# Amandaynzhou/CGC-Net

Hardware: AMD Instinct MI355X
Metric: cell-graphs/sec (fwd+bwd), batch=32, ~1800 nodes/16 feat (higher is better)
Workload: dtype f32; 1 GPU; C3: full CGC-Net (3 conv blocks + 2 DiffPool) fwd+bwd+Adam, 32 graphs/GPU/step, ~1803 nodes, ~16159 edges/graph, 16 feat, max_num_nodes=11404 (C1=1140, C2=114), flags=shipped; global_batch=32, nodes_per_batch=57711, parallelism=dp1, includes=CSR build + fwd + loss + bwd + grad all-reduce + Adam, step_sequencer=True, node_order=draw order, fused_adam=True, optimiser=cgc_adam_step (one launch; torch fused Adam arithmetic)

## Files before the change

cgc-net_amd/csrc/exec.hip:

```cpp
#include <stdio.h>
#include <stdlib.h>
#include <string.h>

#include "common.hpp"
#include "groups.hpp"

struct CatArgs {
  const float* src[4];
  int ld[4], width[4], off[4];
};
__global__ __launch_bounds__(256) void k_cat_cols(float* __restrict__ dst, int ldd, long long rows, int total_w, CatArgs a, int nsrc,
                                                  int accumulate) {
  const long long total = rows * total_w;
  for (long long i = blockIdx.x * 256ll + threadIdx.x; i < total; i += (long long)gridDim.x * 256) {
    const long long r = i / total_w;
    const int c = (int)(i - r * total_w);
    int s = 0;
#pragma unroll
    for (int k = 1; k < 4; ++k)
      if (k < nsrc && c >= a.off[k]) s = k;
    const float v = a.src[s][r * a.ld[s] + (c - a.off[s])];
    float* p = dst + r * ldd + c;
    *p = accumulate ? *p + v : v;
  }
}

extern "C" int cgc_cat_cols(float* dst, int ldd, int rows, int nsrc, const float* const* srcs, const int* lds, const int* widths,
                            int accumulate, cgc_stream_t stream) {
  if (nsrc < 1 || nsrc > 4) return CGC_EINVAL;
  CatArgs a;
  int off = 0;
  for (int k = 0; k < 4; ++k) {
    a.src[k] = k < nsrc ? srcs[k] : nullptr;
    a.ld[k] = k < nsrc ? lds[k] : 0;
    a.width[k] = k < nsrc ? widths[k] : 0;
    a.off[k] = off;
    off += a.width[k];
  }
  if (rows <= 0 || off <= 0) return 0;
  const long long total = (long long)rows * off;
  const long long blocks = (total + 255) / 256;
  hipLaunchKernelGGL(k_cat_cols, dim3((unsigned)(blocks < 4096 ? blocks : 4096)), dim3(256), 0, as_stream(stream), dst, ldd,
                     (long long)rows, off, a, nsrc, accumulate);
  CGC_RETURN_IF_LAUNCH_FAILED();
  return 0;
}

__global__ __launch_bounds__(256) void k_transpose(const float* __restrict__ src, int lds, int rows, int cols, float* __restrict__ dst,
                                                   int ldd) {
  __shared__ float t[32][33];
  const int tx = threadIdx.x & 31, ty = threadIdx.x >> 5;
  const int r0 = blockIdx.y * 32, c0 = blockIdx.x * 32;
  for (int j = ty; j < 32; j += 8) {
    const int r = r0 + j, c = c0 + tx;
    if (r < rows && c < cols) t[j][tx] = src[(size_t)r * lds + c];
  }
  __syncthreads();
  for (int j = ty; j < 32; j += 8) {
    const int c = c0 + j, r = r0 + tx;
    if (r < rows && c < cols) dst[(size_t)c * ldd + r] = t[tx][j];
  }
}

extern "C" int cgc_transpose(const float* src, int lds, int rows, int cols, float* dst, int ldd, cgc_stream_t stream) {
  if (rows <= 0 || cols <= 0) return 0;
  hipLaunchKernelGGL(k_transpose, dim3((unsigned)ceil_div(cols, 32), (unsigned)ceil_div(rows, 32)), dim3(256), 0, as_stream(stream), src,
                     lds, rows, cols, dst, ldd);
  CGC_RETURN_IF_LAUNCH_FAILED();
  return 0;
}

int reduce_batch_sum_rows(const float* ws, float* out, int parts, int rows, int width, int ldo, float beta, hipStream_t stream);

namespace {

struct Arena {
  float* base;
  size_t off = 0, high = 0;
  explicit Arena(float* b) : base(b) {}
  float* f(size_t n) {
    off = (off + 63) & ~(size_t)63;
    float* p = base + off;
    off += n;
    if (off > high) high = off;
    return p;
  }
  int* i(size_t n) { return reinterpret_cast<int*>(f(n)); }
  size_t mark() const { return off; }
  void release(size_t m) { off = m; }
};

struct Ctx {
  cgc_stream_t s;
  bool dry;
  Arena* scratch;
  float* gws;
  int64_t gws_floats;
  int gemm_mode = CGC_GEMM_EXACT;
};

static int fail_at(int rc, const char* what, int line) {
  static const bool verbose = getenv("CGC_EXEC_DEBUG") != nullptr;
  if (verbose) fprintf(stderr, "cgc exec.hip:%d: rc %d from %s\n", line, rc, what);
  return rc;
}
#define CALL(expr)                                              \
  do {                                                          \
    if (!c.dry) {                                               \
      const int rc__ = (expr);                                  \
      if (rc__ != 0) return fail_at(rc__, #expr, __LINE__);     \
    }                                                           \
  } while (0)
#define TRY(expr)                                               \
  do {                                                          \
    const int rc__ = (expr);                                    \
    if (rc__ != 0) return fail_at(rc__, #expr, __LINE__);       \
  } while (0)

inline int up(int v, int m) { return (v + m - 1) / m * m; }
inline int wide_ld(int F) { return (F >= 256 && F % 32 != 0) ? up(F, 32) : (F > 32 && F % 4 != 0) ? up(F, 4) : F; }
inline int pad4_ld(int c) { return (c > 32 && c % 4 != 0) ? up(c, 4) : c; }

int gemm(const Ctx& c, int tA, int tB, int M, int N, int K, const float* A, int lda, const float* B, int ldb, float beta, float* C, int ldc,
         const float* bias = nullptr, int batch = 1, int64_t sA = 0, int64_t sB = 0, int64_t sC = 0, const int* gptr = nullptr,
         int ragged = 0, int max_ragged = 0, int nx = 0, const float* const* xA = nullptr, const int* xlda = nullptr,
         const int64_t* xsA = nullptr, const float* const* xB = nullptr, const int* xldb = nullptr, const int64_t* xsB = nullptr,
         const int* xK = nullptr) {
  if (c.dry) return 0;
  return cgc_gemm_f32(tA, tB, M, N, K, 1.f, A, lda, B, ldb, beta, C, ldc, bias, batch, sA, sB, sC, gptr, ragged, max_ragged, nx, xA, xlda,
                      xsA, xB, xldb, xsB, xK, c.gws, c.gws_floats, c.gemm_mode, c.s);
}

int gemm_x1(const Ctx& c, int tA, int tB, int M, int N, int K, const float* A, int lda, const float* B, int ldb, float beta, float* C, int ldc,
            const float* bias, int batch, int64_t sA, int64_t sB, int64_t sC, const int* gptr, int ragged, int max_ragged, const float* xA,
            int xlda, int64_t xsA, const float* xB, int xldb, int64_t xsB, int xK) {
  return gemm(c, tA, tB, M, N, K, A, lda, B, ldb, beta, C, ldc, bias, batch, sA, sB, sC, gptr, ragged, max_ragged, 1, &xA, &xlda, &xsA,
              &xB, &xldb, &xsB, &xK);
}

int split_parts(int Fa, int Fb, int n) {
  const int tm = Fa <= 32 ? 32 : Fa <= 64 ? 64 : 128, tn = Fb <= 32 ? 32 : Fb <= 64 ? 64 : 128;
  const int tiles = ceil_div(Fa, tm) * ceil_div(Fb, tn);
  int best = 1;
  double best_score = -1.0;
  int hi = n / 512;
  if (hi > 128) hi = 128;
  if (hi < 1) hi = 1;
  for (int parts = 1; parts <= hi; ++parts) {
    const int blocks = tiles * parts, rounds = ceil_div(blocks, 512);
    const double fill = (double)blocks / ((double)rounds * 512.0);
    const double score = fill - 0.02 * rounds - (blocks < 256 ? 0.5 : 0.0);
    if (score > best_score + 1e-9) {
      best = parts;
      best_score = score;
    }
  }
  return best;
}

int gemm_tn_rows(const Ctx& c, const float* A, int lda, int Fa, const float* B, int ldb, int Fb, int n, float* out, int ldo = 0) {
  if (ldo <= 0) ldo = Fb;
  int parts = split_parts(Fa, Fb, n);
  if (parts == 1) return gemm(c, 1, 0, Fa, Fb, n, A, lda, B, ldb, 0.f, out, ldo);
  const int chunk = up(ceil_div(n, parts), 32);
  parts = ceil_div(n, chunk);
  const size_t m = c.scratch->mark();
  float* ws = c.scratch->f((size_t)parts * Fa * Fb);
  TRY(gemm(c, 1, 0, Fa, Fb, n, A, lda, B, ldb, 0.f, ws, Fb, nullptr, parts, 0, 0, (int64_t)Fa * Fb, nullptr, 3, chunk));
  CALL(reduce_batch_sum_rows(ws, out, parts, Fa, Fb, ldo, 0.f, as_stream(c.s)));
  c.scratch->release(m);
  return 0;
}

struct T3 {
  float* p;
  int b, r, c, ld;
  int64_t bs() const { return (int64_t)r * ld; }
};

int bgemm(const Ctx& c, const T3& A, const T3& B, const T3& C, int tA, int tB, float beta = 0.f) {
  const int batch = C.b, M = C.r, N = C.c, Kd = tA ? A.r : A.c;
  if (tA && !tB && M <= 128 && N <= 128 && Kd >= 512 && batch * 2 < 256 && C.ld == N) {
    int parts = Kd / 128;
    const int want = ceil_div(384, batch * (N > 64 ? 2 : 1));
    if (want < parts) parts = want;
    if (parts < 2) parts = 2;
    const int step = up(ceil_div(Kd, parts), 32);
    parts = ceil_div(Kd, step);
    const size_t m = c.scratch->mark();
    float* ws = c.scratch->f((size_t)batch * parts * M * N);
    TRY(gemm(c, 1, 0, M, N, Kd, A.p, A.ld, B.p, B.ld, 0.f, ws, N, nullptr, batch * parts, 0, 0, (int64_t)M * N, nullptr, 3, step));
    CALL(cgc_reduce_batched(ws, C.p, batch, parts, M * N, beta, c.s));
    c.scratch->release(m);
    return 0;
  }
  return gemm(c, tA, tB, M, N, Kd, A.p, A.ld, B.p, B.ld, beta, C.p, C.ld, nullptr, batch, A.bs(), B.bs(), C.bs());
}

int cat2(const Ctx& c, float* dst, int ldd, int rows, const float* a, int lda, int wa, const float* b, int ldb, int wb, int accumulate = 0) {
  const float* s[2] = {a, b};
  const int l[2] = {lda, ldb}, w[2] = {wa, wb};
  CALL(cgc_cat_cols(dst, ldd, rows, 2, s, l, w, accumulate, c.s));
  return 0;
}
int cat3(const Ctx& c, float* dst, int ldd, int rows, const float* a, int lda, int wa, const float* b, int ldb, int wb, const float* d, int ldd3,
         int wd) {
  const float* s[3] = {a, b, d};
  const int l[3] = {lda, ldb, ldd3}, w[3] = {wa, wb, wd};
  CALL(cgc_cat_cols(dst, ldd, rows, 3, s, l, w, 0, c.s));
  return 0;
}
int add1(const Ctx& c, float* dst, int ldd, int rows, const float* a, int lda, int wa) {
  const float* s[1] = {a};
  const int l[1] = {lda}, w[1] = {wa};
  CALL(cgc_cat_cols(dst, ldd, rows, 1, s, l, w, 1, c.s));
  return 0;
}

struct LayerP {
  const float *W, *b, *gamma, *beta;
  float *rm, *rv;
  int64_t* nbt;
  float eps, mom;
};
struct LayerS {
  float *hn, *rinv, *mean, *istd;
};

inline LayerP layer_params(const cgc_level_desc& d, const cgc_block_params* p, int k, int slot) {
  LayerP r;
  r.W = p->W[k];
  r.b = d.has_bias ? p->b[k] : nullptr;
  r.gamma = d.has_bn ? p->gamma[k] : nullptr;
  r.beta = d.has_bn ? p->beta[k] : nullptr;
  r.rm = d.has_bn ? p->running_mean[k] : nullptr;
  r.rv = d.has_bn ? p->running_var[k] : nullptr;
  r.nbt = d.has_bn ? p->num_batches_tracked[k] : nullptr;
  r.eps = d.bn_eps[slot];
  r.mom = d.bn_momentum[slot];
  return r;
}

inline size_t stats_ws_floats(int n, int F) { return (size_t)cgc_stats_ws_floats(n, F); }

int layer_fwd(const Ctx& c, const cgc_level_desc& d, const LayerP& p, const LayerS& s, const float* agg, int lda, int n, int fin, int F,
              float* y, int ldy, float* y2 = nullptr, int ldy2 = 0) {
  const size_t m = c.scratch->mark();
  const int batch_stats = d.has_bn && !d.eval;
  float* ws = batch_stats ? c.scratch->f(stats_ws_floats(n, F)) : nullptr;
  int fused = 0;
  if ((F >= 256 || F <= 32) && fin <= 32 && !c.dry) {
    int rc;
    if (F <= 32)
      rc = cgc_sage_narrow_fwd(agg, lda, p.W, p.b, n, fin, F, 1, d.act, s.hn, s.rinv, batch_stats, ws, d.count, p.eps, p.mom, p.rm, p.rv, p.nbt,
                               s.mean, s.istd, c.s);
    else
      rc = cgc_sage_wide_fwd(agg, lda, p.W, p.b, n, fin, F, 1, d.act, s.hn, F, s.rinv, batch_stats, ws, d.count, p.eps, p.mom, p.rm, p.rv, p.nbt,
                             s.mean, s.istd, c.s);
    if (rc == 0) fused = 1;
    else if (rc != CGC_EINVAL) return rc;
  }
  if (!fused) {
    TRY(gemm(c, 0, 0, n, F, fin, agg, lda, p.W, F, 0.f, s.hn, F, p.b));
    if (batch_stats)
      CALL(cgc_l2norm_act_bn(s.hn, n, F, 1, d.act, s.hn, s.rinv, ws, d.count, p.eps, p.mom, p.rm, p.rv, p.nbt, s.mean, s.istd, c.s));
    else
      CALL(cgc_l2norm_act_stats(s.hn, n, F, 1, d.act, s.hn, s.rinv, nullptr, nullptr, c.s));
  }
  if (d.has_bn && d.eval) CALL(cgc_bn_running_stats(p.rm, p.rv, F, p.eps, s.mean, s.istd, c.s));
  CALL(cgc_bn_act_apply(s.hn, n, F, d.act, d.has_bn ? s.mean : nullptr, s.istd, p.gamma, p.beta, y, ldy, y2, ldy2, c.s));
  c.scratch->release(m);
  return 0;
}

int layer_bwd(const Ctx& c, const cgc_level_desc& d, const LayerP& p, const LayerS& s, const float* agg, int lda, int n, int fin, int F,
              const float* dy, int ldy, float* dagg, int ldd, float* dwdb, float* sums) {
  const size_t m = c.scratch->mark();
  const int mode = d.has_bn ? 2 : 0;
  const size_t slot_floats = (size_t)(cgc_stats_blocks(n, F) > 1 ? cgc_stats_blocks(n, F) : 1) * 2 * F;
  if (d.has_bn) {
    float* ws = c.scratch->f(slot_floats);
    CALL(cgc_bn_bwd_reduce(dy, ldy, s.hn, n, F, d.act, s.mean, s.istd, sums, ws, c.s));
  }
  float* db = d.has_bias ? dwdb + (size_t)fin * F : nullptr;
  if (F <= 32 && fin <= 32) {
    float* ws = c.scratch->f((size_t)cgc_sage_narrow_ws_floats(n, fin, F));
    CALL(cgc_sage_narrow_bwd(dy, ldy, s.hn, s.rinv, n, F, d.act, 1, mode, s.mean, s.istd, p.gamma, d.has_bn ? sums : nullptr, d.count, agg,
                             lda, fin, p.W, dagg, ldd, dwdb, ws, c.s));
  } else {
    float* dh = c.scratch->f((size_t)n * F);
    float* ws = db ? c.scratch->f(slot_floats) : nullptr;
    CALL(cgc_bn_act_l2_bwd(dy, ldy, s.hn, s.rinv, n, F, d.act, 1, mode, s.mean, s.istd, p.gamma, d.has_bn ? sums : nullptr, d.count, dh, db, ws,
                           c.s));
    if (dagg) TRY(gemm(c, 0, 1, n, fin, F, dh, F, p.W, F, 0.f, dagg, ldd));
    TRY(gemm_tn_rows(c, agg, lda, fin, dh, F, F, n, dwdb));
  }
  c.scratch->release(m);
  return 0;
}

inline bool pairable(int fin_e, int F_e, int fin_p, int F_p) { return fin_e == fin_p && F_e == F_p && fin_e <= 32 && F_e <= 32; }

int layer_fwd_pair(const Ctx& c, const cgc_level_desc& d, const LayerP* p, const LayerS* s, const float* const* agg, int lda, int n, int fin, int F,
                   float* const* y, int ldy, float* const* y2, const int* ldy2) {
  const size_t m = c.scratch->mark();
  SnFwdPtrs g[2];
  SnFwdBn bn[2];
  BnApplyPtrs ap[2];
  const int batch_stats = d.has_bn && !d.eval;
  for (int i = 0; i < 2; ++i) {
    float* ws = batch_stats ? c.scratch->f(stats_ws_floats(n, F)) : nullptr;
    g[i] = SnFwdPtrs{agg[i], p[i].W, p[i].b, s[i].hn, s[i].rinv, ws};
    bn[i] = SnFwdBn{p[i].eps, p[i].mom, p[i].rm, p[i].rv, p[i].nbt, s[i].mean, s[i].istd};
    ap[i] = BnApplyPtrs{s[i].hn, d.has_bn ? s[i].mean : nullptr, s[i].istd, p[i].gamma, p[i].beta, y[i], y2[i], ldy2[i]};
  }
  CALL(sage_narrow_fwd_groups(g, bn, 2, lda, n, fin, F, 1, d.act, batch_stats, d.count, as_stream(c.s)));
  if (d.has_bn && d.eval)
    for (int i = 0; i < 2; ++i) CALL(cgc_bn_running_stats(p[i].rm, p[i].rv, F, p[i].eps, s[i].mean, s[i].istd, c.s));
  CALL(bn_act_apply_groups(ap, 2, n, F, d.act, ldy, as_stream(c.s)));
  c.scratch->release(m);
  return 0;
}

int layer_bwd_pair(const Ctx& c, const cgc_level_desc& d, const LayerP* p, const LayerS* s, const float* const* agg, int lda, int n, int fin, int F,
                   const float* const* dy, int ldy, float* const* dagg, int ldd, float* const* dwdb, float* const* sums) {
  const size_t m = c.scratch->mark();
  const int mode = d.has_bn ? 2 : 0;
  const size_t slot_floats = (size_t)(cgc_stats_blocks(n, F) > 1 ? cgc_stats_blocks(n, F) : 1) * 2 * F;
  if (d.has_bn) {
    BnRedPtrs r[2];
    for (int i = 0; i < 2; ++i) r[i] = BnRedPtrs{dy[i], s[i].hn, s[i].mean, s[i].istd, c.scratch->f(slot_floats)};
    CALL(bn_bwd_reduce_groups(r, sums, 2, ldy, n, F, d.act, as_stream(c.s)));
  }
  SnBwdPtrs g[2];
  for (int i = 0; i < 2; ++i)
    g[i] = SnBwdPtrs{dy[i], s[i].hn, s[i].rinv, s[i].mean, s[i].istd, p[i].gamma, d.has_bn ? sums[i] : nullptr, agg[i], p[i].W, dagg[i],
                     c.scratch->f((size_t)cgc_sage_narrow_ws_floats(n, fin, F))};
  CALL(sage_narrow_bwd_groups(g, dwdb, 2, ldy, n, F, d.act, 1, mode, d.count, lda, fin, ldd, as_stream(c.s)));
  c.scratch->release(m);
  return 0;
}

struct Level {
  const cgc_level_desc& d;
  int n, B, R, fin, H, E, AH, C, D, D3, wp, wt, ldp, ldC, ldP, ldW, ftot, npad_jk, seg_nmax;
  bool dense, pool, tall;
  float *At, *An, *invd, *ge1, *agg0, *pair[2], *xcat, *aggk[2], *hp3, *cat_e, *HS, *CS, *jk_out, *x12, *S, *P;
  float *G, *keep;
  bool reg;
  double reg_numel, reg_rows;
  int* arg;
  LayerS L[6];
  cgc_level_grad_layout gl;

  explicit Level(const cgc_level_desc& dd) : d(dd) {
    n = d.n; B = d.B; R = d.rows_per_graph; fin = d.fin; H = d.H; E = d.E; AH = d.AH; C = d.C;
    dense = d.level >= 2;
    pool = C > 0;
    D3 = 2 * H + E;
    D = d.jk ? H : D3;
    wp = pool ? H + AH : H;
    wt = 2 * wp + fin;
    ldp = dense ? wt : wp;
    ldC = pool ? wide_ld(C) : 0;
    ldP = dense ? pad4_ld(C) : ldC;
    ftot = 2 * AH + C;
    tall = pool && n >= 8 * C;
    ldW = wide_ld(C);
    npad_jk = up(n > 1 ? n : 1, 1024);
    seg_nmax = dense ? R : d.npad;
    reg = pool && (d.flags & 8);
    const double N = dense ? R : d.npad;
    reg_numel = (double)B * N * N;
    reg_rows = (double)B * N;
    memset(&gl, 0, sizeof(gl));
  }

  void layout_saved(Arena& a) {
    At = An = invd = ge1 = nullptr;
    if (dense) {
      if (d.renorm) At = a.f((size_t)n * R);
      An = a.f((size_t)n * R);
      invd = a.f(n);
      ge1 = a.f(n);
    }
    agg0 = a.f((size_t)n * fin);
    xcat = dense ? a.f((size_t)n * wt) : nullptr;
    for (int k = 0; k < 2; ++k) {
      pair[k] = dense ? xcat + (1 - k) * wp : a.f((size_t)n * wp);
      aggk[k] = a.f((size_t)n * wp);
    }
    hp3 = pool ? a.f((size_t)n * ldC) : nullptr;
    for (int k = 0; k < 6; ++k) {
      const bool emb = k < 3;
      if (!emb && !pool) {
        L[k].hn = L[k].rinv = L[k].mean = L[k].istd = nullptr;
        continue;
      }
      const int F = width_out(k);
      L[k].hn = a.f((size_t)n * F);
      L[k].rinv = a.f(n);
      L[k].mean = a.f(F);
      L[k].istd = a.f(F);
    }
    cat_e = a.f((size_t)n * D3);
    HS = CS = jk_out = nullptr;
    if (d.jk) {
      const int Hh = 3 * H / 2;
      HS = a.f((size_t)6 * Hh * npad_jk);
      CS = a.f((size_t)6 * Hh * npad_jk);
      jk_out = a.f((size_t)n * H);
    }
    arg = a.i((size_t)B * D);
    x12 = S = P = nullptr;
    if (pool) {
      x12 = a.f((size_t)n * 2 * AH);
      S = a.f((size_t)n * ldC);
      P = a.f((size_t)n * ldP);
    }
    G = keep = nullptr;
    if (reg) {
// ... 84 lines not shown
  TRY(aggregate(c, L, g, gptr, x_in, L.fin, L.fin, L.agg0));
  if (L.dense) {
    const float* s1[1] = {x_in};
    const int l1[1] = {L.fin}, w1[1] = {L.fin};
    CALL(cgc_cat_cols(L.xcat + 2 * wp, L.wt, n, 1, s1, l1, w1, 0, c.s));
  }
  for (int k = 0; k < 3; ++k) {
    const float* ain = k == 0 ? L.agg0 : L.aggk[k - 1];
    const int lda = k == 0 ? L.fin : wp;
    if (k < 2 && L.pool && pairable(L.width_in(k), H, L.width_in(3 + k), AH)) {
      const LayerP pp[2] = {layer_params(d, emb, k, k), layer_params(d, pl, k, 3 + k)};
      const LayerS ss[2] = {L.L[k], L.L[3 + k]};
      const float* ag[2] = {ain, k == 0 ? ain : ain + H};
      float* yy[2] = {L.pair[k], L.pair[k] + H};
      float* y2[2] = {L.cat_e + k * H, L.x12 + k * AH};
      const int l2[2] = {L.D3, 2 * AH};
      TRY(layer_fwd_pair(c, d, pp, ss, ag, lda, n, L.width_in(k), H, yy, L.ldp, y2, l2));
      if (k < 2) TRY(aggregate(c, L, g, gptr, L.pair[k], L.ldp, wp, L.aggk[k]));
      continue;
    }
    if (k < 2)
      TRY(layer_fwd(c, d, layer_params(d, emb, k, k), L.L[k], ain, lda, n, L.width_in(k), L.width_out(k), L.pair[k], L.ldp, L.cat_e + k * H,
                    L.D3));
    else
      TRY(layer_fwd(c, d, layer_params(d, emb, k, k), L.L[k], ain, lda, n, L.width_in(k), L.width_out(k), L.cat_e + 2 * H, L.D3));
    if (L.pool) {
      const float* ainp = k == 0 ? ain : ain + H;
      if (k < 2)
        TRY(layer_fwd(c, d, layer_params(d, pl, k, 3 + k), L.L[3 + k], ainp, lda, n, L.width_in(3 + k), L.width_out(3 + k), L.pair[k] + H, L.ldp,
                      L.x12 + k * AH, 2 * AH));
      else
        TRY(layer_fwd(c, d, layer_params(d, pl, k, 3 + k), L.L[3 + k], ainp, lda, n, L.width_in(3 + k), L.width_out(3 + k), L.hp3, L.ldC));
    }
    if (k < 2) TRY(aggregate(c, L, g, gptr, L.pair[k], L.ldp, wp, L.aggk[k]));
  }
  if (d.jk) CALL(cgc_jk_lstm_fwd(L.cat_e, n, L.npad_jk, H, jk->lstm, jk->w_att, jk->b_att, L.jk_out, L.HS, L.CS, c.s));
  CALL(cgc_segment_max_fwd(L.embed(), gptr, L.B, L.D, L.seg_nmax, readout, L.arg, c.s));
  if (!L.pool) return 0;
  {
    const bool wide_main = C > 2 * AH;
    const float* xm = wide_main ? L.hp3 : L.x12;
    const float* xe = wide_main ? L.x12 : L.hp3;
    const int ldm = wide_main ? L.ldC : 2 * AH, lde = wide_main ? 2 * AH : L.ldC;
    const int wm = wide_main ? C : 2 * AH, we = wide_main ? 2 * AH : C;
    const int om = wide_main ? 2 * AH : 0, oe = wide_main ? 0 : 2 * AH;
    if (L.tall) {
      const size_t m = c.scratch->mark();
      float* wt = c.scratch->f((size_t)L.ftot * L.ldW);
      CALL(cgc_transpose(pl->lin_W, L.ftot, C, L.ftot, wt, L.ldW, c.s));
      TRY(gemm_x1(c, 0, 0, n, C, wm, xm, ldm, wt + (size_t)om * L.ldW, L.ldW, 0.f, L.S, L.ldC, pl->lin_b, 1, 0, 0, 0, nullptr, 0, 0, xe, lde, 0,
                  wt + (size_t)oe * L.ldW, L.ldW, 0, we));
      c.scratch->release(m);
    } else {
      TRY(gemm_x1(c, 0, 1, n, C, wm, xm, ldm, pl->lin_W + om, L.ftot, 0.f, L.S, L.ldC, pl->lin_b, 1, 0, 0, 0, nullptr, 0, 0, xe, lde, 0,
                  pl->lin_W + oe, L.ftot, 0, we));
    }
  }
  CALL(cgc_softmax_fwd(L.S, n, C, L.ldC, L.S, c.s));
  if (!L.dense) {
    CALL(cgc_spmm_graphs(g->rowptr, g->col, nullptr, g->val, nullptr, nullptr, L.S, L.P, n, C, L.ldC, gptr, L.B, d.nmax, 1 | (g->spatial ? 4 : 0), g->gorder, c.s));
    TRY(gemm(c, 1, 0, C, L.D, 0, L.S, L.ldC, L.embed(), L.D, 0.f, x_out, L.D, nullptr, L.B, 0, 0, (int64_t)C * L.D, gptr, 2, d.nmax));
    TRY(gemm(c, 1, 0, C, C, 0, L.S, L.ldC, L.P, L.ldC, 0.f, A_out, C, nullptr, L.B, 0, 0, (int64_t)C * C, gptr, 2, d.nmax));
  } else {
    const T3 s3{L.S, L.B, L.R, C, L.ldC}, e3{const_cast<float*>(L.embed()), L.B, L.R, L.D, L.D}, p3{L.P, L.B, L.R, C, L.ldP};
    const T3 a3{const_cast<float*>(d.renorm ? L.At : A_in), L.B, L.R, L.R, L.R};
    TRY(bgemm(c, s3, e3, T3{x_out, L.B, C, L.D, L.D}, 1, 0));
    TRY(bgemm(c, a3, s3, p3, 0, 0));
    TRY(bgemm(c, s3, p3, T3{A_out, L.B, C, C, C}, 1, 0));
  }
  if (L.reg) TRY(reg_fwd(c, L, g, gptr, A_in, A_out, reg_out));
  return 0;
}

int level_bwd_blocks(const Ctx& c, Level& L, const cgc_block_params* emb, const cgc_block_params* pl, const cgc_jk_params* jk,
                     const cgc_graph* g, const int* gptr, const float* x_in, const float* A_in, float* d_embed, const float* dx12,
                     float* dagg1, const float* gAt, float* grads, float* d_x_in, float* d_A_in) {
  const cgc_level_desc& d = L.d;
  Arena& sc = *c.scratch;
  const int n = L.n, H = L.H, AH = L.AH, wp = L.wp, B = L.B, R = L.R, D3 = L.D3, fin = L.fin;
  auto sums = [&](int k) { return grads + L.gl.W[k] + (int64_t)L.width_in(k) * L.width_out(k) + L.width_out(k); };
  float* d_cat = d_embed;
  if (d.jk) {
    d_cat = sc.f((size_t)n * D3);
    const size_t m = sc.mark();
    float* ws = sc.f((size_t)cgc_jk_bwd_ws_floats(H));
    CALL(cgc_jk_lstm_bwd_flat(L.cat_e, d_embed, n, L.npad_jk, H, jk->lstm, jk->w_att, jk->b_att, L.HS, L.CS, d_cat, grads + L.gl.jk, ws, c.s));
    sc.release(m);
  }
  float* dagg[2];
  const int ldg = L.ldp;
  float* const gcat = dagg1 != nullptr ? dagg1 : sc.f((size_t)n * ldg);
  dagg[1] = gcat;
  TRY(layer_bwd(c, d, layer_params(d, emb, 2, 2), L.L[2], L.aggk[1], wp, n, H, L.E, d_cat + 2 * H, D3, dagg[1], ldg, grads + L.gl.W[2], sums(2)));
  float* dpair = nullptr;
  for (int k = 1; k >= 0; --k) {
    dpair = sc.f((size_t)n * wp);
    TRY(aggregate_t(c, L, g, gptr, dagg[k], ldg, wp, dpair));
    if (L.pool) TRY(cat2(c, dpair, wp, n, d_cat + k * H, D3, H, dx12 + k * AH, 2 * AH, AH, 1));
    else TRY(add1(c, dpair, wp, n, d_cat + k * H, D3, H));
    const bool first = k == 0;
    const bool need_in = !first || L.dense;
    const float* ain = first ? L.agg0 : L.aggk[k - 1];
    const int lda = first ? fin : wp;
    const int fi_e = L.width_in(k), fi_p = L.width_in(3 + k);
    float *de = nullptr, *dp = nullptr;
    int ldd = ldg;
    if (need_in && !first) {
      de = dagg[0] = L.dense ? gcat + wp : sc.f((size_t)n * wp);
      dp = de + H;
    } else if (need_in) {
      de = gcat + 2 * wp;
      dp = L.pool ? sc.f((size_t)n * ldg) : nullptr;
    }
    if (L.pool && pairable(fi_e, H, fi_p, AH)) {
      const LayerP pp[2] = {layer_params(d, emb, k, k), layer_params(d, pl, k, 3 + k)};
      const LayerS ss[2] = {L.L[k], L.L[3 + k]};
      const float* ag[2] = {ain, first ? ain : ain + H};
      const float* dyy[2] = {dpair, dpair + H};
      float* dg[2] = {de, dp};
      float* dw[2] = {grads + L.gl.W[k], grads + L.gl.W[3 + k]};
      float* sm[2] = {sums(k), sums(3 + k)};
      TRY(layer_bwd_pair(c, d, pp, ss, ag, lda, n, fi_e, H, dyy, wp, dg, ldd, dw, sm));
    } else {
      TRY(layer_bwd(c, d, layer_params(d, emb, k, k), L.L[k], ain, lda, n, fi_e, H, dpair, wp, de, ldd, grads + L.gl.W[k], sums(k)));
      if (L.pool)
        TRY(layer_bwd(c, d, layer_params(d, pl, k, 3 + k), L.L[3 + k], first ? ain : ain + H, lda, n, fi_p, AH, dpair + H, wp, dp, ldd,
                      grads + L.gl.W[3 + k], sums(3 + k)));
    }
    if (first && L.dense) {
      if (L.pool) TRY(add1(c, de, ldg, n, dp, ldg, fin));
      TRY(aggregate_t(c, L, g, gptr, de, ldg, fin, d_x_in));
      float* dAn = sc.f((size_t)n * R);
      TRY(bgemm(c, T3{gcat, B, R, L.wt, L.wt}, T3{L.xcat, B, R, L.wt, L.wt}, T3{dAn, B, R, R, R}, 0, 1));
      CALL(cgc_adj_prep_bwd(A_in, L.An, L.invd, L.ge1, dAn, gAt, n, R, d.renorm ? d.renorm_p : -1.f, d_A_in, c.s));
    }
  }
  return 0;
}

int level_bwd(const Ctx& c, Level& L, const cgc_block_params* emb, const cgc_block_params* pl, const cgc_jk_params* jk, const cgc_graph* g,
              const int* gptr, const float* x_in, const float* A_in, const float* d_readout, const float* d_xo, const float* d_ao, float* grads,
              float* d_x_in, float* d_A_in, const float* d_reg = nullptr) {
  const cgc_level_desc& d = L.d;
  Arena& sc = *c.scratch;
  const int n = L.n, H = L.H, AH = L.AH, wp = L.wp, C = L.C, D = L.D, B = L.B, R = L.R;
  float* d_embed = sc.f((size_t)n * D);
  CALL(cgc_segment_max_bwd_full(d_readout, L.arg, gptr, B, D, L.seg_nmax, d_embed, c.s));
  float *dx12 = nullptr, *gAt = nullptr;
  if (L.pool) {
    float *Gs = nullptr, *coef = nullptr;
    if (L.reg) {
      float* dao = sc.f((size_t)B * C * C);
      Gs = sc.f((size_t)B * C * C);
      coef = sc.f(4);
      CALL(cgc_diffpool_reg_bwd_prep(d_reg, L.keep, L.reg_numel, L.reg_rows, d_ao, dao, L.G, Gs, B, C, coef, c.s));
      d_ao = dao;
    }
    const size_t m0 = sc.mark();
    float* ds = sc.f((size_t)n * L.ldC);
    if (!L.dense) {
      float* dp = sc.f((size_t)n * L.ldC);
      TRY(gemm(c, 0, 0, 0, C, C, L.S, L.ldC, d_ao, C, 0.f, dp, L.ldC, nullptr, B, 0, (int64_t)C * C, 0, gptr, 1, d.nmax));
      CALL(cgc_spmm_graphs(g->t_rowptr, g->t_col, nullptr, g->t_val, nullptr, nullptr, dp, ds, n, C, L.ldC, gptr, B, d.nmax, 2 | (g->spatial ? 4 : 0), g->gorder,
                           c.s));
      TRY(gemm_x1(c, 0, 1, 0, C, C, L.P, L.ldC, d_ao, C, 1.f, ds, L.ldC, nullptr, B, 0, (int64_t)C * C, 0, gptr, 1, d.nmax, L.embed(), D, 0, d_xo,
                  D, (int64_t)C * D, D));
      if (L.reg) TRY(gemm(c, 0, 0, 0, C, C, L.S, L.ldC, Gs, C, 1.f, ds, L.ldC, nullptr, B, 0, (int64_t)C * C, 0, gptr, 1, d.nmax));
      TRY(gemm(c, 0, 0, 0, D, C, L.S, L.ldC, d_xo, D, 1.f, d_embed, D, nullptr, B, 0, (int64_t)C * D, 0, gptr, 1, d.nmax));
    } else {
      gAt = sc.f((size_t)n * R);
      float* dP = sc.f((size_t)n * L.ldP);
      const T3 s3{L.S, B, R, C, L.ldC}, e3{const_cast<float*>(L.embed()), B, R, D, D}, p3{L.P, B, R, C, L.ldP};
      const T3 a3{const_cast<float*>(d.renorm ? L.At : A_in), B, R, R, R};
      const T3 dao{const_cast<float*>(d_ao), B, C, C, C}, dxo{const_cast<float*>(d_xo), B, C, D, D};
      const T3 ds3{ds, B, R, C, L.ldC}, dP3{dP, B, R, C, L.ldP};
      TRY(bgemm(c, p3, dao, ds3, 0, 1));
      TRY(bgemm(c, s3, dao, dP3, 0, 0));
      TRY(bgemm(c, dP3, s3, T3{gAt, B, R, R, R}, 0, 1));
      TRY(bgemm(c, a3, dP3, ds3, 1, 0, 1.f));
      TRY(bgemm(c, e3, dxo, ds3, 0, 1, 1.f));
      TRY(bgemm(c, s3, dxo, T3{d_embed, B, R, D, D}, 0, 0, 1.f));
      if (L.reg) {
        TRY(bgemm(c, s3, T3{Gs, B, C, C, C}, ds3, 0, 0, 1.f));
        CALL(cgc_diffpool_reg_adj_bwd(a3.p, (int64_t)n * R, coef, gAt, 1, c.s));
      }
    }
    if (L.reg) CALL(cgc_diffpool_reg_entropy_bwd(L.S, n, C, L.ldC, coef, ds, L.ldC, c.s));
    float* dz = sc.f((size_t)n * L.ldC);
    {
      const size_t m = sc.mark();
      float* ws = sc.f((size_t)(cgc_stats_blocks(n, C) > 1 ? cgc_stats_blocks(n, C) : 1) * 2 * C);
      CALL(cgc_softmax_bwd(L.S, ds, n, C, L.ldC, dz, grads + L.gl.lin_b, ws, c.s));
      sc.release(m);
    }
    dx12 = sc.f((size_t)n * 2 * AH);
    float* dy3 = sc.f((size_t)n * L.ldC);
    TRY(gemm(c, 0, 0, n, 2 * AH, C, dz, L.ldC, pl->lin_W, L.ftot, 0.f, dx12, 2 * AH));
    TRY(gemm(c, 0, 0, n, C, C, dz, L.ldC, pl->lin_W + 2 * AH, L.ftot, 0.f, dy3, L.ldC));
    {
      float* dW = grads + L.gl.lin_W;
      TRY(gemm_tn_rows(c, dz, L.ldC, C, L.x12, 2 * AH, 2 * AH, n, dW, L.ftot));
      TRY(gemm_tn_rows(c, dz, L.ldC, C, L.hp3, L.ldC, C, n, dW + 2 * AH, L.ftot));
    }
    (void)m0;
    float* dagg1 = sc.f((size_t)n * L.ldp);
    TRY(layer_bwd(c, d, layer_params(d, pl, 2, 5), L.L[5], L.aggk[1] + H, wp, n, AH, C, dy3, L.ldC, dagg1 + H, L.ldp, grads + L.gl.W[5],
                  grads + L.gl.W[5] + (int64_t)AH * C + C));
    return level_bwd_blocks(c, L, emb, pl, jk, g, gptr, x_in, A_in, d_embed, dx12, dagg1, gAt, grads, d_x_in, d_A_in);
  }
  return level_bwd_blocks(c, L, emb, pl, jk, g, gptr, x_in, A_in, d_embed, nullptr, nullptr, nullptr, grads, d_x_in, d_A_in);
}

template <class Body>
int run_level(const cgc_level_desc* d, float* saved, float* scratch, cgc_stream_t stream, Body&& body) {
  Level L(*d);
  Arena sv(saved), sc(scratch);
  L.layout_saved(sv);
  L.layout_grads();
  Ctx c{stream, false, &sc, nullptr, cgc_gemm_ws_floats()};
  c.gws = sc.f((size_t)c.gws_floats);
  c.gemm_mode = (d->flags & 2) ? CGC_GEMM_SPLIT_BF16 : (d->flags & 4) ? CGC_GEMM_SPLIT_F16 : CGC_GEMM_EXACT;
  return body(c, L);
}

}

extern "C" int cgc_level_supported(const cgc_level_desc* d) {
  if (d == nullptr || d->level < 1 || d->level > 3 || d->B < 1 || d->B > 65535 || d->n < 1) return 0;
  if (d->fin < 1 || d->H < 1 || d->E < 1 || d->act < 0 || d->act > 3) return 0;
  if (d->level >= 2 && (d->rows_per_graph < 1 || (long long)d->B * d->rows_per_graph != d->n)) return 0;
  if (d->level == 1 && (d->nmax < 1 || d->npad < d->nmax)) return 0;
  if (d->C > 0 && (d->AH < 1 || d->H + d->AH > 256 || (2 * d->AH) % 4 != 0)) return 0;
  if (d->C == 0 && d->level == 1) return 0;
  if ((d->flags & ~14) || (d->flags & 6) == 6) return 0;
  if ((d->flags & 8) && d->C == 0) return 0;
  if (d->jk && (d->E != d->H || !cgc_jk_matrix_core(d->H))) return 0;
  return 1;
}

extern "C" int64_t cgc_level_saved_floats(const cgc_level_desc* d) {
  if (!cgc_level_supported(d)) return -1;
  Level L(*d);
  Arena a(nullptr);
  L.layout_saved(a);
  return (int64_t)a.high + 64;
}

extern "C" int cgc_level_grad_layout_of(const cgc_level_desc* d, cgc_level_grad_layout* out) {
  if (!cgc_level_supported(d) || out == nullptr) return CGC_EINVAL;
  Level L(*d);
  L.layout_grads();
  *out = L.gl;
  return 0;
}

extern "C" int64_t cgc_level_scratch_floats(const cgc_level_desc* d) {
  if (!cgc_level_supported(d)) return -1;
  Level L(*d);
  Arena sv(nullptr);
  L.layout_saved(sv);
  L.layout_grads();
  size_t high = 0;
  for (int pass = 0; pass < (d->eval ? 1 : 2); ++pass) {
    Arena sc(nullptr);
    Ctx c{nullptr, true, &sc, nullptr, 0};
    sc.f((size_t)cgc_gemm_ws_floats());
    cgc_block_params bp;
    memset(&bp, 0, sizeof(bp));
    cgc_jk_params jp;
    memset(&jp, 0, sizeof(jp));
    cgc_graph gr;
    memset(&gr, 0, sizeof(gr));
    const int rc = pass == 0 ? level_fwd(c, L, &bp, &bp, &jp, &gr, nullptr, nullptr, nullptr, nullptr, nullptr, nullptr)
                             : level_bwd(c, L, &bp, &bp, &jp, &gr, nullptr, nullptr, nullptr, nullptr, nullptr, nullptr, nullptr, nullptr, nullptr);
    if (rc != 0) return -1;
    if (sc.high > high) high = sc.high;
  }
  return (int64_t)high + 64;
}

extern "C" int cgc_level_fwd(const cgc_level_desc* d, const cgc_block_params* emb, const cgc_block_params* pool, const cgc_jk_params* jk,
                             const cgc_graph* g, const int* gptr, const float* x_in, const float* A_in, float* saved, float* scratch,
                             float* readout, float* x_out, float* A_out, const float** assign_out, int* assign_ld, float* reg_out,
                             cgc_stream_t stream) {
  if (!cgc_level_supported(d) || saved == nullptr || scratch == nullptr) return CGC_EINVAL;
  if (!aligned16(saved) || !aligned16(scratch)) return CGC_EINVAL;
  if ((d->flags & 8) && reg_out == nullptr) return CGC_EINVAL;
  return run_level(d, saved, scratch, stream, [&](const Ctx& c, Level& L) {
    const int rc = level_fwd(c, L, emb, pool, jk, g, gptr, x_in, A_in, readout, x_out, A_out, reg_out);
    if (assign_out != nullptr) *assign_out = L.S;
    if (assign_ld != nullptr) *assign_ld = L.ldC;
    return rc;
  });
}

extern "C" int cgc_level_bwd(const cgc_level_desc* d, const cgc_block_params* emb, const cgc_block_params* pool, const cgc_jk_params* jk,
                             const cgc_graph* g, const int* gptr, const float* x_in, const float* A_in, const float* saved, float* scratch,
                             const float* d_readout, const float* d_x_out, const float* d_A_out, const float* d_reg, float* grads,
                             float* d_x_in, float* d_A_in, cgc_stream_t stream) {
  if (!cgc_level_supported(d) || saved == nullptr || scratch == nullptr || grads == nullptr || d->eval) return CGC_EINVAL;
  if (!aligned16(saved) || !aligned16(scratch) || !aligned16(grads)) return CGC_EINVAL;
  if ((d->flags & 8) && d_reg == nullptr) return CGC_EINVAL;
  return run_level(d, const_cast<float*>(saved), scratch, stream, [&](const Ctx& c, Level& L) {
    return level_bwd(c, L, emb, pool, jk, g, gptr, x_in, A_in, d_readout, d_x_out, d_A_out, grads, d_x_in, d_A_in, d_reg);
  });
}
```

cgc-net_amd/csrc/gemm.hip:

```cpp
#include "gemm_common.hpp"

template <int ROWS>
struct KContigLoader {
  static constexpr int UNITS = ROWS * (BK / 4);
  static constexpr int PER_T = (UNITS + 255) / 256;
  float4 reg[PER_T];
  __device__ __forceinline__ void load(const float* __restrict__ base, int ld, int row0, int row_lim, int k0, int k_lim, bool vec_ok) {
#pragma unroll
    for (int i = 0; i < PER_T; ++i) {
      const int u = threadIdx.x + i * 256;
      float4 v = make_float4(0.f, 0.f, 0.f, 0.f);
      if (UNITS % 256 == 0 || u < UNITS) {
        const int row = row0 + u / (BK / 4);
        const int k = k0 + (u % (BK / 4)) * 4;
        if (row < row_lim && k < k_lim) {
          const float* p = base + (size_t)row * ld + k;
          if (vec_ok && k + 3 < k_lim) {
            v = *reinterpret_cast<const float4*>(p);
          } else {
            v.x = p[0];
            if (k + 1 < k_lim) v.y = p[1];
            if (k + 2 < k_lim) v.z = p[2];
            if (k + 3 < k_lim) v.w = p[3];
          }
        }
      }
      reg[i] = v;
    }
  }
  __device__ __forceinline__ void load_fast(const float* __restrict__ base, int ld, int row0, int row_last, int k0) {
#pragma unroll
    for (int i = 0; i < PER_T; ++i) {
      const int u = threadIdx.x + i * 256;
      const int row = min(row0 + u / (BK / 4), row_last);
      reg[i] = *reinterpret_cast<const float4*>(base + (size_t)row * ld + k0 + (u % (BK / 4)) * 4);
    }
  }
  __device__ __forceinline__ void offsets(unsigned (&off)[PER_T], int ld, int row0, int row_last) const {
#pragma unroll
    for (int i = 0; i < PER_T; ++i) {
      const int u = threadIdx.x + i * 256;
      off[i] = (unsigned)min(row0 + u / (BK / 4), row_last) * (unsigned)ld * 4u + (unsigned)(u % (BK / 4)) * 16u;
    }
  }
  static __device__ __forceinline__ unsigned tile_soffset(int , int k0) { return (unsigned)k0 * 4u; }
  __device__ __forceinline__ void load_buf_part(int i, __amdgpu_buffer_rsrc_t rsrc, const unsigned (&off)[PER_T], unsigned soff) {
    reg[i] = __builtin_bit_cast(float4, __builtin_amdgcn_raw_buffer_load_b128(rsrc, off[i], soff, 0));
  }
  __device__ __forceinline__ void load_fast_masked(const float* __restrict__ base, int ld, int row0, int row_last, int k0, int k_lim) {
    const int k_last4 = (k_lim - 1) & ~3;
#pragma unroll
    for (int i = 0; i < PER_T; ++i) {
      const int u = threadIdx.x + i * 256;
      const int row = min(row0 + u / (BK / 4), row_last);
      const int k = k0 + (u % (BK / 4)) * 4;
      float4 v = *reinterpret_cast<const float4*>(base + (size_t)row * ld + min(k, k_last4));
      if (k >= k_lim) v.x = 0.f;
      if (k + 1 >= k_lim) v.y = 0.f;
      if (k + 2 >= k_lim) v.z = 0.f;
      if (k + 3 >= k_lim) v.w = 0.f;
      reg[i] = v;
    }
  }
  __device__ __forceinline__ void store_part(int i, float* __restrict__ lds) const {
    const int u = threadIdx.x + i * 256;
    if (UNITS % 256 == 0 || u < UNITS)
      *reinterpret_cast<float4*>(&lds[(u / (BK / 4)) * KC_LD + (u % (BK / 4)) * 4]) = reg[i];
  }
  __device__ __forceinline__ void store(float* __restrict__ lds) const {
#pragma unroll
    for (int i = 0; i < PER_T; ++i) store_part(i, lds);
  }
};

template <int COLS>
struct MnContigLoader {
  static constexpr int UNITS = BK * (COLS / 4);
  static constexpr int PER_T = (UNITS + 255) / 256;
  float4 reg[PER_T];
  __device__ __forceinline__ void load(const float* __restrict__ base, int ld, int col0, int col_lim, int k0, int k_lim, bool vec_ok) {
#pragma unroll
    for (int i = 0; i < PER_T; ++i) {
      const int u = threadIdx.x + i * 256;
// ... 484 lines not shown
  if (batch <= 0 || N <= 0) return 0;
  if (ragged == 1 && (transA || a.gptr == nullptr)) return CGC_EINVAL;
  if (ragged == 2 && (!transA || transB || a.gptr == nullptr || a.nx > 0)) return CGC_EINVAL;
  if (ragged == 3 && (!transA || transB || a.nx > 0 || max_ragged <= 0 || K <= 0 || batch % ceil_div(K, max_ragged) != 0)) return CGC_EINVAL;
  if (ragged < 0 || ragged > 3) return CGC_EINVAL;
  a.chunk = ragged == 3 ? max_ragged : 0;
  const int m_extent = ragged == 1 ? max_ragged : M;
  if (m_extent <= 0) return 0;
  const int k_extent = ragged >= 2 ? max_ragged : K;
  constexpr int shortk_max = 160, fill_min = 448;
  const bool sk = k_extent <= shortk_max && a.nx == 0;
  const long long fill = (long long)ceil_div(m_extent, 128) * batch;
  const bool want_split = mode == CGC_GEMM_SPLIT_BF16, want_half = mode == CGC_GEMM_SPLIT_F16;
  auto big_route = [&](bool shortk, float* w) -> int {
    if ((want_split || want_half) && !shortk && !(transA && transB) && gemm_all_fast(a, transA, transB, batch, m_extent, k_extent)) {
      int rc = want_half ? gemm_half_launch(a, transA, transB, batch, m_extent, k_extent, w, ws_floats, stream) : CGC_EINVAL;
      if (rc == CGC_EINVAL) rc = gemm_split_launch(a, transA, transB, batch, m_extent, k_extent, w, ws_floats, stream);
      if (rc != CGC_EINVAL) return rc;
    }
    return launch_cfg<2, 2, 2, 2>(a, transA, transB, batch, m_extent, k_extent, shortk, w, ws_floats, stream);
  };
  const int force = g_force_cfg;
  if (force > 0) {
    const bool fsk = force >= 20 ? true : force >= 10 ? false : sk;
    switch (force % 10) {
      case 1: return big_route(fsk, ws);
      case 2: return launch_cfg<4, 1, 1, 2>(a, transA, transB, batch, m_extent, k_extent, fsk, ws, ws_floats, stream);
      case 3: return launch_cfg<1, 4, 2, 1>(a, transA, transB, batch, m_extent, k_extent, fsk, ws, ws_floats, stream);
      case 4: return launch_cfg<2, 2, 1, 1>(a, transA, transB, batch, m_extent, k_extent, fsk, ws, ws_floats, stream);
      case 5: return launch_cfg<4, 1, 1, 1>(a, transA, transB, batch, m_extent, k_extent, fsk, ws, ws_floats, stream);
      case 6: return launch_cfg<1, 4, 1, 1>(a, transA, transB, batch, m_extent, k_extent, fsk, ws, ws_floats, stream);
      default: break;
    }
  }
  if (N <= 32) return launch_cfg<4, 1, 1, 1>(a, transA, transB, batch, m_extent, k_extent, sk, ws, ws_floats, stream);
  if (N <= 64) {
    if (m_extent > 64 && fill < fill_min) return launch_cfg<2, 2, 1, 1>(a, transA, transB, batch, m_extent, k_extent, sk, ws, ws_floats, stream);
    return launch_cfg<4, 1, 1, 2>(a, transA, transB, batch, m_extent, k_extent, sk, ws, ws_floats, stream);
  }
  if (m_extent <= 32) return launch_cfg<1, 4, 1, 1>(a, transA, transB, batch, m_extent, k_extent, sk, ws, ws_floats, stream);
  if (m_extent <= 64) return launch_cfg<1, 4, 2, 1>(a, transA, transB, batch, m_extent, k_extent, sk, ws, ws_floats, stream);
  if (fill * ceil_div(N, 128) < fill_min) {
    if (N <= 128) {
      if (k_extent > 256 && m_extent > 128)
        return launch_cfg<4, 1, 1, 1>(a, transA, transB, batch, m_extent, k_extent, sk, ws, ws_floats, stream);
      return launch_cfg<2, 2, 1, 1>(a, transA, transB, batch, m_extent, k_extent, sk, ws, ws_floats, stream);
    }
    if (transA) {
      if (!sk && ws != nullptr && k_extent >= 24 * BK) return big_route(sk, ws);
      return launch_cfg<4, 1, 1, 2>(a, transA, transB, batch, m_extent, k_extent, sk, ws, ws_floats, stream);
    }
    return launch_cfg<1, 4, 2, 1>(a, transA, transB, batch, m_extent, k_extent, sk, ws, ws_floats, stream);
  }
  return big_route(sk, ws);
}

extern "C" int cgc_gemm_f32(int transA, int transB, int M, int N, int K, float alpha, const float* A, int lda, const float* B, int ldb,
                            float beta, float* C, int ldc, const float* bias, int batch, int64_t strideA, int64_t strideB,
                            int64_t strideC, const int* gptr, int ragged, int max_ragged, int nx, const float* const* xA,
                            const int* xlda, const int64_t* xstrideA, const float* const* xB, const int* xldb,
                            const int64_t* xstrideB, const int* xK, float* ws, int64_t ws_floats, int mode, cgc_stream_t stream_) {
  if (nx < 0 || nx > 2) return CGC_EINVAL;
  if (mode != CGC_GEMM_EXACT && mode != CGC_GEMM_SPLIT_BF16 && mode != CGC_GEMM_SPLIT_F16) return CGC_EINVAL;
  GemmArgs a;
  a.A = A; a.B = B; a.C = C; a.bias = bias; a.gptr = gptr;
  a.M = M; a.N = N; a.K = K; a.lda = lda; a.ldb = ldb; a.ldc = ldc;
  a.strideA = strideA; a.strideB = strideB; a.strideC = strideC;
  a.alpha = alpha; a.beta = beta; a.ragged = ragged; a.tiles_n = 0;
  a.per_batch = a.nb = 0; a.ws = nullptr; a.resident = 0; a.s_max = 1; a.chunk = 0; a.scale = nullptr;
  for (int i = 0; i < 2; ++i) { a.xA[i] = a.xB[i] = nullptr; a.xlda[i] = a.xldb[i] = a.xK[i] = 0; a.xsA[i] = a.xsB[i] = 0; }
  int kept = 0;
  for (int i = 0; i < nx; ++i) {
    if (xK[i] <= 0) continue;
    a.xA[kept] = xA[i]; a.xB[kept] = xB[i]; a.xlda[kept] = xlda[i]; a.xldb[kept] = xldb[i]; a.xK[kept] = xK[i];
    a.xsA[kept] = xstrideA[i]; a.xsB[kept] = xstrideB[i];
    ++kept;
  }
  a.nx = kept;
  return gemm_dispatch(a, transA, transB, batch, max_ragged, ws, ws_floats, mode, as_stream(stream_));
}

__global__ void k_reduce_batch_sum(const float* __restrict__ ws, float* __restrict__ out, int parts, long long numel, float beta, int width,
                                   int ldo) {
  for (long long i = blockIdx.x * (long long)blockDim.x + threadIdx.x; i < numel; i += (long long)gridDim.x * blockDim.x) {
    float s = 0.f;
    for (int p = 0; p < parts; ++p) s += ws[(size_t)p * numel + i];
    const long long o = (i / width) * ldo + i % width;
    out[o] = beta != 0.f ? s + beta * out[o] : s;
  }
}

__global__ __launch_bounds__(256) void k_reduce_many_parts(const float* __restrict__ ws, float* __restrict__ out, int parts, int numel,
                                                           float beta, int width, int ldo) {
  __shared__ float part[8][32];
  const int cl = threadIdx.x & 31, grp = threadIdx.x >> 5;
  const int c = blockIdx.x * 32 + cl;
  ws += (size_t)blockIdx.y * parts * numel;
  out += (size_t)blockIdx.y * numel;
  float s = 0.f;
  if (c < numel) {
    float a[8];
#pragma unroll
    for (int u = 0; u < 8; ++u) a[u] = 0.f;
    int k = grp;
    for (; k + 56 < parts; k += 64) {
#pragma unroll
      for (int u = 0; u < 8; ++u) a[u] += ws[(size_t)(k + 8 * u) * numel + c];
    }
    for (; k < parts; k += 8) a[0] += ws[(size_t)k * numel + c];
    s = ((a[0] + a[1]) + (a[2] + a[3])) + ((a[4] + a[5]) + (a[6] + a[7]));
  }
  part[grp][cl] = s;
  __syncthreads();
  if (grp == 0 && c < numel) {
    float t = part[0][cl];
#pragma unroll
    for (int g = 1; g < 8; ++g) t += part[g][cl];
    const int o = (c / width) * ldo + c % width;
    out[o] = beta != 0.f ? t + beta * out[o] : t;
  }
}

extern "C" int cgc_reduce_batched(const float* ws, float* out, int outer, int parts, int numel, float beta, cgc_stream_t stream) {
  if (numel <= 0 || outer <= 0) return 0;
  if (outer > 65535) return CGC_EINVAL;
  hipLaunchKernelGGL(k_reduce_many_parts, dim3((unsigned)ceil_div(numel, 32), (unsigned)outer), dim3(256), 0, as_stream(stream), ws, out,
                     parts, numel, beta, numel, numel);
  CGC_RETURN_IF_LAUNCH_FAILED();
  return 0;
}

int reduce_batch_sum_rows(const float* ws, float* out, int parts, int rows, int width, int ldo, float beta, hipStream_t stream) {
  const int64_t numel = (int64_t)rows * width;
  if (numel <= 0) return 0;
  if (width <= 0 || ldo < width || numel > 0x7fffffff) return CGC_EINVAL;
  if (parts >= 16 && numel <= (1 << 20)) {
    hipLaunchKernelGGL(k_reduce_many_parts, dim3((unsigned)ceil_div((int)numel, 32), 1u), dim3(256), 0, stream, ws, out, parts, (int)numel, beta,
                       width, ldo);
  } else {
    const int64_t blocks = ceil_div64(numel, 256);
    hipLaunchKernelGGL(k_reduce_batch_sum, dim3((unsigned)(blocks < 4096 ? blocks : 4096)), dim3(256), 0, stream, ws, out, parts,
                       (long long)numel, beta, width, ldo);
  }
  CGC_RETURN_IF_LAUNCH_FAILED();
  return 0;
}

extern "C" int cgc_reduce_batch_sum(const float* ws, float* out, int parts, int64_t numel, float beta, cgc_stream_t stream) {
  if (numel <= 0) return 0;
  if (parts >= 16 && numel <= (1 << 20)) return cgc_reduce_batched(ws, out, 1, parts, (int)numel, beta, stream);
  const int64_t blocks = ceil_div64(numel, 256);
  const int w = numel <= 0x7fffffff ? (int)numel : 0x7fffffff;
  hipLaunchKernelGGL(k_reduce_batch_sum, dim3((unsigned)(blocks < 4096 ? blocks : 4096)), dim3(256), 0, as_stream(stream), ws, out,
                     parts, (long long)numel, beta, w, w);
  CGC_RETURN_IF_LAUNCH_FAILED();
  return 0;
}
```

cgc-net_amd/csrc/groups.hpp:

```cpp
#pragma once
#include "common.hpp"

struct SnFwdPtrs {
  const float *agg, *W, *bias;
  float *hn, *rinv, *ws;
};
struct SnFwdBn {
  float eps, momentum;
  float *running_mean, *running_var;
  int64_t* nbt;
  float *mean, *istd;
};
struct SnBwdPtrs {
  const float *dy, *hn, *rinv, *mean, *istd, *gamma, *sums, *agg, *W;
  float *dagg, *ws;
};
struct StatsFinPtrs {
  const float* ws;
  float *running_mean, *running_var, *mean, *istd;
  long long* nbt;
  float eps, momentum;
};
struct BnApplyPtrs {
  const float *hn, *mean, *istd, *gamma, *beta;
  float *y, *y2;
  int ldy2;
};
struct BnRedPtrs {
  const float *dy, *hn, *mean, *istd;
  float* ws;
};

int sage_narrow_fwd_groups(const SnFwdPtrs* g, const SnFwdBn* bn, int ng, int lda, int n, int K, int F, int normalize, int act, int stats,
                           double count, hipStream_t st);
int sage_narrow_bwd_groups(const SnBwdPtrs* g, float* const* dwdb, int ng, int ldy, int n, int F, int act, int normalize, int mode, double count,
                           int lda, int fin, int ldd, hipStream_t st);
int bn_act_apply_groups(const BnApplyPtrs* g, int ng, int n, int F, int act, int ldy, hipStream_t stream);
int bn_bwd_reduce_groups(const BnRedPtrs* g, float* const* sums, int ng, int ldy, int n, int F, int act, hipStream_t stream);
int launch_stats_finalize_groups(const StatsFinPtrs* g, int ng, int slots, int F, double count, hipStream_t stream);
int launch_reduce_slots_f32_pair(const float* ws0, float* out0, const float* ws1, float* out1, int ng, int slots, int width, hipStream_t stream);
```

cgc-net_amd/csrc/jk.hip:

```cpp
#include "jk.hpp"

template <int C>
__device__ __forceinline__ void jk_fill_lds(const JkWeights& w, float4* Wt, float4* B4, float* watt, int nthreads) {
  constexpr int H = JkDims<C>::H, KIN = JkDims<C>::KIN;
  for (int idx = threadIdx.x; idx < 2 * H * KIN; idx += nthreads) {
    const int d = idx / (H * KIN), rem = idx - d * H * KIN, j = rem / KIN, k = rem - j * KIN;
    float v[4];
#pragma unroll
    for (int g = 0; g < 4; ++g) {
      const int row = g * H + j;
      v[g] = k < C ? w.w_ih[d][row * C + k] : w.w_hh[d][row * H + (k - C)];
    }
    Wt[idx] = make_float4(v[0], v[1], v[2], v[3]);
  }
  for (int idx = threadIdx.x; idx < 2 * H; idx += nthreads) {
    const int d = idx / H, j = idx - d * H;
    float v[4];
#pragma unroll
    for (int g = 0; g < 4; ++g) v[g] = w.b_ih[d][g * H + j] + w.b_hh[d][g * H + j];
    B4[idx] = make_float4(v[0], v[1], v[2], v[3]);
    watt[idx] = w.w_att[idx];
  }
  if (threadIdx.x == 0) watt[2 * H] = w.b_att[0];
}
// ... 255 lines not shown
extern "C" int cgc_jk_matrix_core(int C) { return C == 4 || C == 8 || C == 12 || C == 16 || C == 20; }

#define JK_FOR_EACH_C(X) X(2) X(4) X(6) X(8) X(10) X(12) X(14) X(16) X(18) X(20) X(22) X(24) X(26) X(28) X(30) X(32)

template <int C>
static void jk_allow_lds() {
  static bool done_f[CGC_MAX_DEVICES] = {}, done_b[CGC_MAX_DEVICES] = {};
  cgc_allow_lds(reinterpret_cast<const void*>(&k_jk_fwd<C>), (int)JkDims<C>::lds_bytes, done_f);
  cgc_allow_lds(reinterpret_cast<const void*>(&k_jk_bwd<C>), (int)JkDims<C>::lds_bytes, done_b);
}

template <int C>
static int launch_jk_fwd(const float* xs, int n, int npad, const JkWeights& w, float* out, float* HS, float* CS, hipStream_t st) {
  jk_allow_lds<C>();
  hipLaunchKernelGGL(k_jk_fwd<C>, dim3(ceil_div(2 * n, JK_THREADS)), dim3(JK_THREADS), JkDims<C>::lds_bytes, st, xs, n, npad, w, out, HS, CS);
  CGC_RETURN_IF_LAUNCH_FAILED();
  return 0;
}
template <int C>
static int launch_jk_bwd(const float* xs, const float* dout, int n, int npad, const JkWeights& w, const float* HS, const float* CS,
                         float* dxs, float* DGT, float* INT, float* DHC, hipStream_t st) {
  jk_allow_lds<C>();
  hipLaunchKernelGGL(k_jk_bwd<C>, dim3(ceil_div(2 * npad, JK_THREADS)), dim3(JK_THREADS), JkDims<C>::lds_bytes, st, xs, dout, n, npad, w,
                     HS, CS, dxs, DGT, INT, DHC);
  CGC_RETURN_IF_LAUNCH_FAILED();
  return 0;
}

extern "C" int cgc_jk_lstm_fwd(const float* xs, int n, int npad, int C, const float* const* lstm, const float* w_att,
                               const float* b_att, float* out, float* HS, float* CS, cgc_stream_t stream) {
  if (n <= 0) return 0;
  if (!jk_npad_ok(n, npad)) return CGC_EINVAL;
  JkWeights w;
  fill_weights(w, lstm, w_att, b_att);
  const int rc = jk_mfma_fwd(xs, n, npad, C, w, out, HS, CS, as_stream(stream));
  if (rc != CGC_EINVAL) return rc;
  switch (C) {
#define X(C_) case C_: return launch_jk_fwd<C_>(xs, n, npad, w, out, HS, CS, as_stream(stream));
    JK_FOR_EACH_C(X)
#undef X
    default: return CGC_EINVAL;
  }
}

extern "C" int cgc_jk_lstm_bwd(const float* xs, const float* dout, int n, int npad, int C, const float* const* lstm,
                               const float* w_att, const float* b_att, const float* HS, const float* CS, float* dxs, float* DGT,
                               float* INT, float* DHC, cgc_stream_t stream) {
  if (n <= 0) return 0;
  if (!jk_npad_ok(n, npad)) return CGC_EINVAL;
  JkWeights w;
  fill_weights(w, lstm, w_att, b_att);
  const int rc = jk_mfma_bwd(xs, dout, n, npad, C, w, HS, CS, dxs, DGT, INT, as_stream(stream));
  if (rc != CGC_EINVAL) return rc;
  switch (C) {
#define X(C_) case C_: return launch_jk_bwd<C_>(xs, dout, n, npad, w, HS, CS, dxs, DGT, INT, DHC, as_stream(stream));
    JK_FOR_EACH_C(X)
#undef X
    default: return CGC_EINVAL;
  }
}

extern "C" int64_t cgc_jk_bwd_ws_floats(int C) { return jk_mfma_bwd_ws_floats(C); }

extern "C" int cgc_jk_lstm_bwd_params(const float* xs, const float* dout, int n, int npad, int C, const float* const* lstm,
                                      const float* w_att, const float* b_att, const float* HS, const float* CS, float* dxs,
                                      float* G, float* ws, cgc_stream_t stream) {
  if (n <= 0) return 0;
  if (!jk_npad_ok(n, npad)) return CGC_EINVAL;
  JkWeights w;
  fill_weights(w, lstm, w_att, b_att);
  return jk_mfma_bwd_params(xs, dout, n, npad, C, w, HS, CS, dxs, G, ws, as_stream(stream));
}

extern "C" int cgc_jk_lstm_bwd_flat(const float* xs, const float* dout, int n, int npad, int C, const float* const* lstm,
                                    const float* w_att, const float* b_att, const float* HS, const float* CS, float* dxs,
                                    float* flat, float* ws, cgc_stream_t stream) {
  if (n <= 0) return 0;
  if (!jk_npad_ok(n, npad)) return CGC_EINVAL;
  JkWeights w;
  fill_weights(w, lstm, w_att, b_att);
  return jk_mfma_bwd_flat(xs, dout, n, npad, C, w, HS, CS, dxs, flat, ws, as_stream(stream));
}

__global__ void k_jk_unpack(const float* __restrict__ G, int C, int H, float* __restrict__ flat) {
  const int NI = C + 2 * H + 1, NG = 4 * H + 1;
  const int per_dir = 4 * H * C + 4 * H * H + 8 * H, total = 2 * per_dir + 2 * H + 1;
  for (int i = blockIdx.x * blockDim.x + threadIdx.x; i < total; i += gridDim.x * blockDim.x) {
    float v;
    if (i < 2 * per_dir) {
      const int d = i / per_dir;
      int e = i - d * per_dir;
      const float* Gd = G + (size_t)d * NG * NI;
      if (e < 4 * H * C) v = Gd[(e / C) * NI + (e % C)];
      else if ((e -= 4 * H * C) < 4 * H * H) v = Gd[(e / H) * NI + C + (e % H)];
      else { e -= 4 * H * H; v = Gd[(e % (4 * H)) * NI + C + H]; }
    } else {
      const int e = i - 2 * per_dir;
      if (e < 2 * H) v = G[((size_t)(e / H) * NG + 4 * H) * NI + C + H + 1 + (e % H)];
      else v = G[(size_t)(4 * H) * NI + C + H];
    }
    flat[i] = v;
  }
}

extern "C" int64_t cgc_jk_param_grad_floats(int C) {
  const int64_t H = 3 * (int64_t)C / 2;
  return 2 * (4 * H * C + 4 * H * H + 8 * H) + 2 * H + 1;
}

extern "C" int cgc_jk_unpack_param_grads(const float* G, int C, float* flat, cgc_stream_t stream) {
  if (C <= 0) return CGC_EINVAL;
  const int H = 3 * C / 2;
  const int total = (int)cgc_jk_param_grad_floats(C);
  hipLaunchKernelGGL(k_jk_unpack, dim3(ceil_div(total, 256)), dim3(256), 0, as_stream(stream), G, C, H, flat);
  CGC_RETURN_IF_LAUNCH_FAILED();
  return 0;
}
```

cgc-net_amd/csrc/jk.hpp:

```cpp
#pragma once
#include "common.hpp"

__device__ __forceinline__ float sigmoidf_(float x) { return 1.f / (1.f + expf(-x)); }

template <int C>
struct JkDims {
  static constexpr int H = 3 * C / 2;
  static constexpr int KIN = C + H;
  static constexpr size_t lds_bytes = sizeof(float4) * (2 * H * KIN + 2 * H) + sizeof(float) * (2 * H + 4);
};

struct JkWeights {
  const float* w_ih[2];
  const float* w_hh[2];
  const float* b_ih[2];
  const float* b_hh[2];
  const float* w_att;
  const float* b_att;
};


int jk_mfma_fwd(const float* xs, int n, int npad, int C, const JkWeights& w, float* out, float* HS, float* CS, hipStream_t st);
int jk_mfma_bwd(const float* xs, const float* dout, int n, int npad, int C, const JkWeights& w, const float* HS, const float* CS,
                float* dxs, float* DGT, float* INT, hipStream_t st);
int64_t jk_mfma_bwd_ws_floats(int C);
int jk_mfma_bwd_params(const float* xs, const float* dout, int n, int npad, int C, const JkWeights& w, const float* HS,
                       const float* CS, float* dxs, float* G, float* ws, hipStream_t st);
int jk_mfma_bwd_flat(const float* xs, const float* dout, int n, int npad, int C, const JkWeights& w, const float* HS, const float* CS,
                     float* dxs, float* flat, float* ws, hipStream_t st);
```

cgc-net_amd/csrc/jk_mfma.hip:

```cpp
#include "jk.hpp"

typedef float floatx16 __attribute__((ext_vector_type(16)));

constexpr int JKB_TILES = 2;
constexpr int JKB_THREADS = JKB_TILES * 128;

template <int C>
struct JkM {
  static constexpr int H = 3 * C / 2;
  static constexpr int XG = (C + 7) / 8;
  static constexpr int HG = (H + 7) / 8;
  static constexpr int NQ = XG + HG;
  static constexpr int W_FLOATS = 2 * 4 * NQ * 32 * 8;
  static constexpr int B_OFF = W_FLOATS;
  static constexpr int A_OFF = B_OFF + 2 * 4 * 32;
  static constexpr int S_OFF = A_OFF + 2 * 32 + 4;
  static constexpr int TOTAL = S_OFF + 2 * 2 * 3 * 32;
  static_assert(H <= 32 && C % 4 == 0, "one 32-row tile per gate; 16-byte x fragments");
};

__device__ __forceinline__ float jk_rcp(float d) {
  const float r = __builtin_amdgcn_rcpf(d);
  return fmaf(fmaf(-d, r, 1.f), r, r);
}
__device__ __forceinline__ float jk_exp(float a) {
  const float t = a * 0x1.715476p+0f;
  const float r = fmaf(a, 0x1.4ae0cp-26f, fmaf(a, 0x1.715476p+0f, -t));
  const float e = __builtin_amdgcn_exp2f(t);
  return fmaf(e, t >= 16.f ? r * 0x1.62e43p-1f : 0.f, e);
}
__device__ __forceinline__ float fast_sigmoid(float x) { return jk_rcp(1.f + jk_exp(fminf(-x, 87.f))); }
__device__ __forceinline__ float fast_tanh(float x) {
  const float ax = fabsf(x), x2 = x * x;
  const float e = __expf(-2.f * ax);
  const float big = (1.f - e) * jk_rcp(1.f + e);
  const float small = ax * fmaf(x2, fmaf(x2, fmaf(x2, fmaf(x2, 62.f / 2835.f, -17.f / 315.f), 2.f / 15.f), -1.f / 3.f), 1.f);
  return copysignf(ax < 0.25f ? small : big, x);
}

template <int C>
__device__ __forceinline__ void jkm_fill(const JkWeights& w, float* lds, int nthreads) {
  using M = JkM<C>;
  constexpr int H = M::H, XG = M::XG, NQ = M::NQ;
  {
    const int tt = threadIdx.x & 3, lhi = (threadIdx.x >> 2) & 1, j = (threadIdx.x >> 3) & 31;
    float v[2 * 4 * NQ];
#pragma unroll
    for (int it = 0; it < 2 * 4 * NQ; ++it) {
      const int q = it % NQ, g = (it / NQ) & 3, d = it / (4 * NQ);
      v[it] = 0.f;
      if (q < XG) {
        const int k = 8 * q + 4 * lhi + tt;
        if (j < H && k < C) v[it] = w.w_ih[d][(g * H + j) * C + k];
      } else {
        const int k = 8 * (q - XG) + 4 * lhi + tt;
        if (j < H && k < H) v[it] = w.w_hh[d][(g * H + j) * H + k];
      }
    }
#pragma unroll
    for (int it = 0; it < 2 * 4 * NQ; ++it) lds[it * 256 + threadIdx.x] = v[it];
  }
  for (int idx = threadIdx.x; idx < 2 * 4 * 32; idx += nthreads) {
    const int j = idx & 31, g = (idx >> 5) & 3, d = idx >> 7;
    lds[M::B_OFF + idx] = j < H ? w.b_ih[d][g * H + j] + w.b_hh[d][g * H + j] : 0.f;
  }
  for (int idx = threadIdx.x; idx < 2 * 32; idx += nthreads) {
    const int j = idx & 31, d = idx >> 5;
    lds[M::A_OFF + idx] = j < H ? w.w_att[d * H + j] : 0.f;
  }
  if (threadIdx.x == 0) lds[M::A_OFF + 64] = w.b_att[0];
}

template <int C>
__global__ __launch_bounds__(JKB_THREADS) void k_jk_bwd_mfma(const float* __restrict__ xs, const float* __restrict__ dout, int n, int npad,
                                                     const JkWeights w, const float* __restrict__ HS, const float* __restrict__ CS,
                                                     float* __restrict__ dxs, float* __restrict__ DGT, float* __restrict__ INT,
                                                     float* __restrict__ ) {
  using M = JkM<C>;
  constexpr int H = M::H, XG = M::XG, HG = M::HG, NQ = M::NQ;
  constexpr int NG = 4 * H + 1, NI = C + 2 * H + 1;
  extern __shared__ __attribute__((aligned(16))) float lds[];
  if (threadIdx.x < 256) jkm_fill<C>(w, lds, 256);
  __syncthreads();
// ... 144 lines not shown
#pragma unroll
      for (int q = 0; q < XG; ++q) {
        if (8 * q + 4 * lhi < C) {
          inT[(size_t)(8 * q + 4 * lhi + 0) * ktot + col] = xt[q].x;
          inT[(size_t)(8 * q + 4 * lhi + 1) * ktot + col] = xt[q].y;
          inT[(size_t)(8 * q + 4 * lhi + 2) * ktot + col] = xt[q].z;
          inT[(size_t)(8 * q + 4 * lhi + 3) * ktot + col] = xt[q].w;
        }
      }
#pragma unroll
      for (int q = 0; q < HG; ++q) {
        const float4 wa = *reinterpret_cast<const float4*>(Al + 8 * q);
        const float was[4] = {wa.x, wa.y, wa.z, wa.w};
#pragma unroll
        for (int u = 0; u < 4; ++u) {
          const int r = 4 * q + u, j = u + 8 * q + 4 * lhi;
          const float gi = fast_sigmoid(acc[0][r]), gf = fast_sigmoid(acc[1][r]);
          const float gg = fast_tanh(acc[2][r]), go = fast_sigmoid(acc[3][r]);
          const float c = gf * cprev[r] + gi * gg;
          const float th = fast_tanh(c);
          const float dh = fmaf(dst, was[u], dhc[r]);
          const float dc = fmaf(dh * go, 1.f - th * th, dcc[r]);
          dcc[r] = dc * gf;
          const float qi = dc * gg * gi * (1.f - gi), qf = dc * cprev[r] * gf * (1.f - gf);
          const float qg = dc * gi * (1.f - gg * gg), qo = dh * th * go * (1.f - go);
          acc[0][r] = qi; acc[1][r] = qf; acc[2][r] = qg; acc[3][r] = qo;
          if (8 * q + u < H && j < H) {
            dgt[(size_t)(0 * H + j) * ktot + col] = qi;
            dgt[(size_t)(1 * H + j) * ktot + col] = qf;
            dgt[(size_t)(2 * H + j) * ktot + col] = qg;
            dgt[(size_t)(3 * H + j) * ktot + col] = qo;
            inT[(size_t)(C + j) * ktot + col] = hprev[r];
            inT[(size_t)(C + H + 1 + j) * ktot + col] = go * th;
          }
        }
      }
      floatx16 dh2, dx2;
#pragma unroll
      for (int r = 0; r < 16; ++r) { dh2[r] = 0.f; dx2[r] = 0.f; }
#pragma unroll
      for (int g = 0; g < 4; ++g)
#pragma unroll
        for (int q = 0; q < HG; ++q) {
          float ah[4], ax[4];
#pragma unroll
          for (int u = 0; u < 4; ++u) {
            ax[u] = WtX[g * NQ * 256 + (8 * q + u) * 8];
            ah[u] = s > 0 ? WtH[g * NQ * 256 + (8 * q + u) * 8] : 0.f;
          }
#pragma unroll
          for (int u = 0; u < 4; ++u) {
            dx2 = __builtin_amdgcn_mfma_f32_32x32x2f32(ax[u], acc[g][4 * q + u], dx2, 0, 0, 0);
            if (s > 0) dh2 = __builtin_amdgcn_mfma_f32_32x32x2f32(ah[u], acc[g][4 * q + u], dh2, 0, 0, 0);
          }
        }
      if (s > 0) dhc = dh2;
#pragma unroll
      for (int q = 0; q < XG; ++q) Ex[(t * XG + q) * 64] = make_float4(dx2[4 * q + 0], dx2[4 * q + 1], dx2[4 * q + 2], dx2[4 * q + 3]);
    }

    __syncthreads();
    if (d == 0 && valid) {
      const float4* Eo = Ex + 3 * XG * 64;
#pragma unroll
      for (int q = 0; q < XG; ++q) {
        if (8 * q + 4 * lhi < C) {
          const float4 dy = *reinterpret_cast<const float4*>(dout + (size_t)node * C + 8 * q + 4 * lhi);
#pragma unroll
          for (int t = 0; t < 3; ++t) {
            const float4 p0 = Ex[(t * XG + q) * 64], p1 = Eo[(t * XG + q) * 64];
            float4 v;
            v.x = fmaf(a3[t], dy.x, p0.x + p1.x); v.y = fmaf(a3[t], dy.y, p0.y + p1.y);
            v.z = fmaf(a3[t], dy.z, p0.z + p1.z); v.w = fmaf(a3[t], dy.w, p0.w + p1.w);
            *reinterpret_cast<float4*>(dxs + (size_t)node * 3 * C + t * C + 8 * q + 4 * lhi) = v;
          }
        }
      }
    }
    __syncthreads();
  }
}

__global__ void k_jk_pg_fold(const float* __restrict__ part, int P, int P2, int per, float* __restrict__ tmp) {
  const int e = blockIdx.x * blockDim.x + threadIdx.x, p2 = blockIdx.y, d = blockIdx.z;
  if (e >= per) return;
  const float* src = part + ((size_t)d * P + (size_t)p2 * 16) * per + e;
  const int cnt = min(16, P - p2 * 16);
  float a = 0.f;
  for (int k = 0; k < cnt; ++k) a += src[(size_t)k * per];
  tmp[((size_t)d * P2 + p2) * per + e] = a;
}

template <int C>
struct JkU {
  static constexpr int H = 3 * C / 2, XG = (C + 7) / 8, HG = (H + 7) / 8, NQ = XG + HG;
  static constexpr int W_FLOATS = 2 * 4 * NQ * 256;
  static constexpr int B_OFF = W_FLOATS;
  static constexpr int A_OFF = B_OFF + 256;
  static constexpr int S_OFF = A_OFF + 68;
  static constexpr int X_OFF = S_OFF + 768;
  static constexpr int FWD_TOTAL = X_OFF + 2 * 8 * 256;
  static constexpr int Q_OFF = S_OFF + 768;
  static constexpr int I_OFF = Q_OFF + 8 * 1152;
  static constexpr int P_OFF = I_OFF + 4 * 1152;
  static constexpr int BWD_TOTAL = P_OFF + 8 * XG * 256;
  static constexpr int PG_SLOTS = 37;
  static constexpr int PG_FLOATS = 8 * PG_SLOTS * 64;
  static_assert(H <= 30 && C % 4 == 0, "column 31 of the h tile is the bias column; 16-byte x fragments");
};

template <int C>
__device__ __forceinline__ void jku_fill(const JkWeights& w, float* lds) {
  using U = JkU<C>;
  constexpr int H = U::H, XG = U::XG, NQ = U::NQ;
  const int tid = threadIdx.x, d = tid >> 8;
  const float* wih = d ? w.w_ih[1] : w.w_ih[0];
  const float* whh = d ? w.w_hh[1] : w.w_hh[0];
  const float* bih = d ? w.b_ih[1] : w.b_ih[0];
  const float* bhh = d ? w.b_hh[1] : w.b_hh[0];
  const int tt = tid & 3, lhi = (tid >> 2) & 1, rho = (tid >> 3) & 31, g = rho >> 3, u = rho & 7;
  float v[4 * NQ];
#pragma unroll
  for (int it = 0; it < 4 * NQ; ++it) {
    const int q = it % NQ, ww = it / NQ, j = 8 * ww + u;
    const int jr = j < H ? j : H - 1;
    if (q < XG) {
      const int k = 8 * q + 4 * lhi + tt;
      const float ld = wih[(g * H + jr) * C + (k < C ? k : C - 1)];
      v[it] = (j < H && k < C) ? ld : 0.f;
    } else {
      const int k = 8 * (q - XG) + 4 * lhi + tt;
      const float ld = whh[(g * H + jr) * H + (k < H ? k : H - 1)];
      v[it] = (j < H && k < H) ? ld : 0.f;
    }
  }
#pragma unroll
  for (int it = 0; it < 4 * NQ; ++it) lds[(d * 4 * NQ + it) * 256 + (tid & 255)] = v[it];
  if ((tid & 255) < 128) {
    const int r2 = tid & 31, ww = (tid >> 5) & 3, j = 8 * ww + (r2 & 7), gg = r2 >> 3;
    lds[U::B_OFF + (d * 4 + ww) * 32 + r2] = j < H ? bih[gg * H + j] + bhh[gg * H + j] : 0.f;
  } else if ((tid & 255) < 160) {
    const int j = tid & 31;
    lds[U::A_OFF + d * 32 + j] = j < H ? w.w_att[d * H + j] : 0.f;
  }
  if (tid == 0) lds[U::A_OFF + 64] = w.b_att[0];
}

template <int C>
__global__ __launch_bounds__(512) void k_jku_fwd(const float* __restrict__ xs, int n, int npad, const JkWeights w,
                                                 float* __restrict__ out, float* __restrict__ HS, float* __restrict__ CS) {
  using U = JkU<C>;
  constexpr int H = U::H, XG = U::XG, HG = U::HG, NQ = U::NQ;
  extern __shared__ __attribute__((aligned(16))) float lds[];
  jku_fill<C>(w, lds);
  __syncthreads();
  const int lane = threadIdx.x & 63, l31 = lane & 31, lhi = lane >> 5;
  const int wave = __builtin_amdgcn_readfirstlane(threadIdx.x >> 6), d = wave & 1, ww = wave >> 1;
  const float4* Wl = reinterpret_cast<const float4*>(lds) + (size_t)(d * 4 + ww) * NQ * 64 + l31 * 2 + lhi;
  const float* Bl = lds + U::B_OFF + (d * 4 + ww) * 32 + 4 * lhi;
  const float4 wa4 = *reinterpret_cast<const float4*>(lds + U::A_OFF + d * 32 + 8 * ww + 4 * lhi);
  const float was[4] = {wa4.x, wa4.y, wa4.z, wa4.w};
  float* Sx = lds + U::S_OFF;
  float4* Hx = reinterpret_cast<float4*>(lds + U::X_OFF);
  const int ntiles = (n + 31) / 32;

  for (int tile = blockIdx.x; tile < ntiles; tile += gridDim.x) {
    const int node = tile * 32 + l31;
    const bool valid = node < n, keep = node < npad;
    const float* xrow = xs + (size_t)(valid ? node : 0) * 3 * C + 4 * lhi;
    float cst[4] = {0.f, 0.f, 0.f, 0.f};
    float4 hq[HG];
#pragma unroll
    for (int q = 0; q < HG; ++q) hq[q] = make_float4(0.f, 0.f, 0.f, 0.f);
// ... 380 lines not shown
    for (int k = 0; k < P2; ++k) a += tmp[(size_t)k * per + e];
  } else {
    for (int k = 0; k < P2; ++k) a += tmp[(size_t)k * per + 36 * 64];
  }
  return a;
}

template <int C>
__global__ void k_jku_finish_flat(const float* __restrict__ tmp, int P2, float* __restrict__ flat) {
  constexpr int H = JkU<C>::H;
  constexpr int per_dir = 4 * H * C + 4 * H * H + 8 * H, total = 2 * per_dir + 2 * H + 1;
  const int i = blockIdx.x * blockDim.x + threadIdx.x;
  if (i >= total) return;
  int d, row = 0, col = 0, att = -1;
  if (i < 2 * per_dir) {
    d = i / per_dir;
    int e = i - d * per_dir;
    if (e < 4 * H * C) { row = e / C; col = e % C; }
    else if ((e -= 4 * H * C) < 4 * H * H) { row = e / H; col = C + e % H; }
    else { e -= 4 * H * H; row = e % (4 * H); col = C + H; }
  } else {
    const int e = i - 2 * per_dir;
    if (e < 2 * H) { d = e / H; att = e % H; }
    else { d = 0; att = H; }
  }
  flat[i] = jku_gather<C>(tmp, P2, d, row, col, att);
}

template <int C>
__global__ void k_jku_finish_G(const float* __restrict__ tmp, int P2, float* __restrict__ G) {
  constexpr int H = JkU<C>::H, NG = 4 * H + 1, NI = C + 2 * H + 1;
  const int i = blockIdx.x * blockDim.x + threadIdx.x;
  if (i >= 2 * NG * NI) return;
  const int d = i / (NG * NI), e = i - d * NG * NI, row = e / NI, col = e - row * NI;
  float v = 0.f;
  if (row < 4 * H) {
    if (col <= C + H) v = jku_gather<C>(tmp, P2, d, row, col, -1);
  } else if (col > C + H) {
    v = jku_gather<C>(tmp, P2, d, 0, 0, col - (C + H + 1));
  } else if (col == C + H && d == 0) {
    v = jku_gather<C>(tmp, P2, 0, 0, 0, H);
  }
  G[i] = v;
}

template <int C>
static int launch_fwd(const float* xs, int n, int npad, const JkWeights& w, float* out, float* HS, float* CS, hipStream_t st) {
  constexpr size_t lds = sizeof(float) * JkU<C>::FWD_TOTAL;
  static bool attr_set[CGC_MAX_DEVICES] = {};
  cgc_allow_lds(reinterpret_cast<const void*>(&k_jku_fwd<C>), (int)lds, attr_set);
  int grid = ceil_div(n, 32);
  if (grid > 512) grid = 512;
  hipLaunchKernelGGL(k_jku_fwd<C>, dim3(grid), dim3(512), lds, st, xs, n, npad, w, out, HS, CS);
  CGC_RETURN_IF_LAUNCH_FAILED();
  return 0;
}

int jk_mfma_fwd(const float* xs, int n, int npad, int C, const JkWeights& w, float* out, float* HS, float* CS, hipStream_t st) {
  if ((reinterpret_cast<uintptr_t>(xs) & 15u) || (reinterpret_cast<uintptr_t>(out) & 15u)) return CGC_EINVAL;
  switch (C) {
    case 4: return launch_fwd<4>(xs, n, npad, w, out, HS, CS, st);
    case 8: return launch_fwd<8>(xs, n, npad, w, out, HS, CS, st);
    case 12: return launch_fwd<12>(xs, n, npad, w, out, HS, CS, st);
    case 16: return launch_fwd<16>(xs, n, npad, w, out, HS, CS, st);
    case 20: return launch_fwd<20>(xs, n, npad, w, out, HS, CS, st);
    default: return CGC_EINVAL;
  }
}

template <int C>
static int launch_bwd(const float* xs, const float* dout, int n, int npad, const JkWeights& w, const float* HS, const float* CS,
                      float* dxs, float* DGT, float* INT, hipStream_t st) {
  const size_t lds = sizeof(float) * (JkM<C>::TOTAL + JKB_TILES * 192) + sizeof(float4) * JKB_TILES * 2 * 3 * JkM<C>::XG * 64;
  static bool attr_set[CGC_MAX_DEVICES] = {};
  cgc_allow_lds(reinterpret_cast<const void*>(&k_jk_bwd_mfma<C>), (int)lds, attr_set);
  int grid = ceil_div(npad / 32, JKB_TILES);
  if (grid > 256) grid = 256;
  hipLaunchKernelGGL(k_jk_bwd_mfma<C>, dim3(grid), dim3(JKB_THREADS), lds, st, xs, dout, n, npad, w, HS, CS, dxs, DGT, INT, nullptr);
  CGC_RETURN_IF_LAUNCH_FAILED();
  return 0;
}

template <int C>
static int launch_bwd_params(const float* xs, const float* dout, int n, int npad, const JkWeights& w, const float* HS, const float* CS,
                             float* dxs, float* G, float* ws, hipStream_t st, float* flat) {
  constexpr size_t lds = sizeof(float) * JkU<C>::BWD_TOTAL;
  static bool attr_set[CGC_MAX_DEVICES] = {};
  cgc_allow_lds(reinterpret_cast<const void*>(&k_jku_bwd<C>), (int)lds, attr_set);
  int grid = ceil_div(n, 32);
  if (grid > 256) grid = 256;
  hipLaunchKernelGGL(k_jku_bwd<C>, dim3(grid), dim3(512), lds, st, xs, dout, n, npad, w, HS, CS, dxs, ws);
  CGC_RETURN_IF_LAUNCH_FAILED();
  constexpr int per = JkU<C>::PG_FLOATS, H = JkU<C>::H;
  const int P = grid, P2 = ceil_div(P, 16);
  float* tmp = ws + (size_t)P * per;
  hipLaunchKernelGGL(k_jk_pg_fold, dim3(ceil_div(per, 256), P2, 1), dim3(256), 0, st, ws, P, P2, per, tmp);
  if (flat != nullptr) {
    constexpr int total = 2 * (4 * H * C + 4 * H * H + 8 * H) + 2 * H + 1;
    hipLaunchKernelGGL(k_jku_finish_flat<C>, dim3(ceil_div(total, 128)), dim3(128), 0, st, tmp, P2, flat);
  } else {
    constexpr int total = 2 * (4 * H + 1) * (C + 2 * H + 1);
    hipLaunchKernelGGL(k_jku_finish_G<C>, dim3(ceil_div(total, 128)), dim3(128), 0, st, tmp, P2, G);
  }
  CGC_RETURN_IF_LAUNCH_FAILED();
  return 0;
}

int jk_mfma_bwd(const float* xs, const float* dout, int n, int npad, int C, const JkWeights& w, const float* HS, const float* CS,
                float* dxs, float* DGT, float* INT, hipStream_t st) {
  if ((reinterpret_cast<uintptr_t>(xs) & 15u) || (reinterpret_cast<uintptr_t>(dout) & 15u) || (reinterpret_cast<uintptr_t>(dxs) & 15u) ||
      npad % (32 * JKB_TILES) != 0)
    return CGC_EINVAL;
  switch (C) {
    case 4: return launch_bwd<4>(xs, dout, n, npad, w, HS, CS, dxs, DGT, INT, st);
    case 8: return launch_bwd<8>(xs, dout, n, npad, w, HS, CS, dxs, DGT, INT, st);
    case 12: return launch_bwd<12>(xs, dout, n, npad, w, HS, CS, dxs, DGT, INT, st);
    case 16: return launch_bwd<16>(xs, dout, n, npad, w, HS, CS, dxs, DGT, INT, st);
    case 20: return launch_bwd<20>(xs, dout, n, npad, w, HS, CS, dxs, DGT, INT, st);
    default: return CGC_EINVAL;
  }
}

int64_t jk_mfma_bwd_ws_floats(int C) {
  const int64_t per = (8 * 16 + 16 + 1) * 64;
  (void)C;
  return 2 * 512 * per + 2 * 32 * per;
}

int jk_mfma_bwd_flat(const float* xs, const float* dout, int n, int npad, int C, const JkWeights& w, const float* HS, const float* CS,
                     float* dxs, float* flat, float* ws, hipStream_t st) {
  if ((reinterpret_cast<uintptr_t>(xs) & 15u) || (reinterpret_cast<uintptr_t>(dout) & 15u) || (reinterpret_cast<uintptr_t>(dxs) & 15u))
    return CGC_EINVAL;
  switch (C) {
    case 4: return launch_bwd_params<4>(xs, dout, n, npad, w, HS, CS, dxs, nullptr, ws, st, flat);
    case 8: return launch_bwd_params<8>(xs, dout, n, npad, w, HS, CS, dxs, nullptr, ws, st, flat);
    case 12: return launch_bwd_params<12>(xs, dout, n, npad, w, HS, CS, dxs, nullptr, ws, st, flat);
    case 16: return launch_bwd_params<16>(xs, dout, n, npad, w, HS, CS, dxs, nullptr, ws, st, flat);
    case 20: return launch_bwd_params<20>(xs, dout, n, npad, w, HS, CS, dxs, nullptr, ws, st, flat);
    default: return CGC_EINVAL;
  }
}

int jk_mfma_bwd_params(const float* xs, const float* dout, int n, int npad, int C, const JkWeights& w, const float* HS,
                       const float* CS, float* dxs, float* G, float* ws, hipStream_t st) {
  if ((reinterpret_cast<uintptr_t>(xs) & 15u) || (reinterpret_cast<uintptr_t>(dout) & 15u) || (reinterpret_cast<uintptr_t>(dxs) & 15u))
    return CGC_EINVAL;
  switch (C) {
    case 4: return launch_bwd_params<4>(xs, dout, n, npad, w, HS, CS, dxs, G, ws, st, nullptr);
    case 8: return launch_bwd_params<8>(xs, dout, n, npad, w, HS, CS, dxs, G, ws, st, nullptr);
    case 12: return launch_bwd_params<12>(xs, dout, n, npad, w, HS, CS, dxs, G, ws, st, nullptr);
    case 16: return launch_bwd_params<16>(xs, dout, n, npad, w, HS, CS, dxs, G, ws, st, nullptr);
    case 20: return launch_bwd_params<20>(xs, dout, n, npad, w, HS, CS, dxs, G, ws, st, nullptr);
    default: return CGC_EINVAL;
  }
}
```

cgc-net_amd/csrc/rowops.hip:

```cpp
#include <type_traits>

#include "common.hpp"
#include "groups.hpp"

#define L2_EPS 1e-12f
#define RENORM_EPS 1e-15f
#define MAX_SLOTS 1024

template <int VEC, int MAXJ, int NQ>
__device__ __forceinline__ void col_reduce_store(float (&acc)[NQ][MAXJ][VEC], int F, int lpr, float* smem, float* slot) {
  const int lane = threadIdx.x & 63, wave = threadIdx.x >> 6;
#pragma unroll
  for (int q = 0; q < NQ; ++q)
#pragma unroll
    for (int j = 0; j < MAXJ; ++j)
#pragma unroll
      for (int v = 0; v < VEC; ++v)
        for (int o = 32; o >= lpr; o >>= 1) acc[q][j][v] += __shfl_xor(acc[q][j][v], o);
  if (wave > 0 && lane < lpr) {
#pragma unroll
    for (int q = 0; q < NQ; ++q)
#pragma unroll
      for (int j = 0; j < MAXJ; ++j)
#pragma unroll
        for (int v = 0; v < VEC; ++v) {
          const int c = (lane + lpr * j) * VEC + v;
          if (c < F) smem[((wave - 1) * NQ + q) * F + c] = acc[q][j][v];
        }
  }
  __syncthreads();
  if (wave == 0 && lane < lpr) {
#pragma unroll
    for (int q = 0; q < NQ; ++q)
#pragma unroll
      for (int j = 0; j < MAXJ; ++j)
#pragma unroll
        for (int v = 0; v < VEC; ++v) {
          const int c = (lane + lpr * j) * VEC + v;
          if (c < F) {
            float t = acc[q][j][v];
            for (int w = 0; w < 3; ++w) t += smem[(w * NQ + q) * F + c];
            slot[q * F + c] = t;
          }
        }
  }
}

template <int VEC, int MAXJ>
__device__ __forceinline__ void col_reduce_store_f64(double (&acc)[2][MAXJ][VEC], int F, int lpr, double* smem, double* slot) {
  const int lane = threadIdx.x & 63, wave = threadIdx.x >> 6;
#pragma unroll
  for (int q = 0; q < 2; ++q) {
#pragma unroll
    for (int j = 0; j < MAXJ; ++j)
#pragma unroll
      for (int v = 0; v < VEC; ++v)
        for (int o = 32; o >= lpr; o >>= 1) acc[q][j][v] += __shfl_xor(acc[q][j][v], o);
    if (q > 0) __syncthreads();
    if (wave > 0 && lane < lpr) {
#pragma unroll
      for (int j = 0; j < MAXJ; ++j)
#pragma unroll
        for (int v = 0; v < VEC; ++v) {
          const int c = (lane + lpr * j) * VEC + v;
          if (c < F) smem[(wave - 1) * F + c] = acc[q][j][v];
        }
    }
    __syncthreads();
    if (wave == 0 && lane < lpr) {
#pragma unroll
      for (int j = 0; j < MAXJ; ++j)
#pragma unroll
        for (int v = 0; v < VEC; ++v) {
          const int c = (lane + lpr * j) * VEC + v;
          if (c < F) {
            double t = acc[q][j][v];
            for (int w = 0; w < 3; ++w) t += smem[w * F + c];
            slot[q * F + c] = t;
          }
        }
    }
  }
}

#define RS_GROUPS 32
template <typename OUT, typename IN = float>
__global__ __launch_bounds__(32 * RS_GROUPS) void k_reduce_slots(const IN* __restrict__ ws, int slots, int width, OUT* __restrict__ out) {
  __shared__ double part[RS_GROUPS][32];
  const int cl = threadIdx.x & 31, grp = threadIdx.x >> 5;
  const int c = blockIdx.x * 32 + cl;
  double s = 0.0;
  if (c < width) {
    double a[4] = {0.0, 0.0, 0.0, 0.0};
    int k = grp;
    for (; k + 3 * RS_GROUPS < slots; k += 4 * RS_GROUPS) {
#pragma unroll
      for (int u = 0; u < 4; ++u) a[u] += (double)ws[(size_t)(k + RS_GROUPS * u) * width + c];
    }
    for (; k < slots; k += RS_GROUPS) a[0] += (double)ws[(size_t)k * width + c];
    s = (a[0] + a[1]) + (a[2] + a[3]);
  }
  part[grp][cl] = s;
  __syncthreads();
  if (grp == 0 && c < width) {
    double t[4] = {0.0, 0.0, 0.0, 0.0};
#pragma unroll
    for (int g = 0; g < RS_GROUPS; g += 4) { t[0] += part[g][cl]; t[1] += part[g + 1][cl]; t[2] += part[g + 2][cl]; t[3] += part[g + 3][cl]; }
    out[c] = (OUT)((t[0] + t[1]) + (t[2] + t[3]));
  }
}
#define REDUCE_SLOTS_GRID(width) dim3(ceil_div((width), 32))

__global__ __launch_bounds__(32 * RS_GROUPS) void k_reduce_slots_pair(const float* __restrict__ ws0, float* __restrict__ out0,
                                                                     const float* __restrict__ ws1, float* __restrict__ out1, int slots, int width) {
  const float* __restrict__ ws = blockIdx.y ? ws1 : ws0;
  float* __restrict__ out = blockIdx.y ? out1 : out0;
  __shared__ double part[RS_GROUPS][32];
  const int cl = threadIdx.x & 31, grp = threadIdx.x >> 5;
  const int c = blockIdx.x * 32 + cl;
  double s = 0.0;
  if (c < width) {
    double a[4] = {0.0, 0.0, 0.0, 0.0};
    int k = grp;
    for (; k + 3 * RS_GROUPS < slots; k += 4 * RS_GROUPS) {
#pragma unroll
      for (int u = 0; u < 4; ++u) a[u] += (double)ws[(size_t)(k + RS_GROUPS * u) * width + c];
    }
    for (; k < slots; k += RS_GROUPS) a[0] += (double)ws[(size_t)k * width + c];
    s = (a[0] + a[1]) + (a[2] + a[3]);
  }
  part[grp][cl] = s;
  __syncthreads();
  if (grp == 0 && c < width) {
    double t[4] = {0.0, 0.0, 0.0, 0.0};
#pragma unroll
    for (int g = 0; g < RS_GROUPS; g += 4) { t[0] += part[g][cl]; t[1] += part[g + 1][cl]; t[2] += part[g + 2][cl]; t[3] += part[g + 3][cl]; }
    out[c] = (float)((t[0] + t[1]) + (t[2] + t[3]));
  }
}
int launch_reduce_slots_f32_pair(const float* ws0, float* out0, const float* ws1, float* out1, int ng, int slots, int width, hipStream_t stream) {
  hipLaunchKernelGGL(k_reduce_slots_pair, dim3(ceil_div(width, 32), ng), dim3(32 * RS_GROUPS), 0, stream, ws0, out0, ws1, out1, slots, width);
  CGC_RETURN_IF_LAUNCH_FAILED();
  return 0;
}

int launch_reduce_slots_f32(const float* ws, int slots, int width, float* out, hipStream_t stream) {
  hipLaunchKernelGGL(k_reduce_slots<float>, REDUCE_SLOTS_GRID(width), dim3(32 * RS_GROUPS), 0, stream, ws, slots, width, out);
  CGC_RETURN_IF_LAUNCH_FAILED();
  return 0;
}

struct ColCfg {
  int vec, maxj, lpr, blocks;
  bool ok;
};
static ColCfg col_cfg(int n, int F, bool vec_ok) {
  ColCfg c;
  c.vec = vec_ok ? 4 : 1;
  c.ok = true;
  int chunks = F / c.vec;
  if (chunks <= 64) {
    c.maxj = 1;
    c.lpr = pick_lpr(chunks);
  } else {
    c.lpr = 64;
    int need = ceil_div(chunks, 64);
    if (c.vec == 4 && need > 8) {
      c.vec = 1;
      need = ceil_div(F, 64);
    }
    c.ok = need <= 32;
    c.maxj = need <= 2 ? 2 : need <= 4 ? 4 : (need == 5 && c.vec == 4) ? 5 : need <= 8 ? 8 : need <= 16 ? 16 : 32;
  }
  c.blocks = row_blocks(n, c.lpr, MAX_SLOTS);
  return c;
}

#define DISPATCH_COL(KERNEL, cfg, smem_bytes, stream, ...)                                                   \
  do {                                                                                                       \
    dim3 g__((cfg).blocks), b__(CGC_BLOCK);                                                                  \
    if ((cfg).vec == 4) {                                                                                    \
      switch ((cfg).maxj) {                                                                                  \
        case 1: hipLaunchKernelGGL((KERNEL<4, 1>), g__, b__, smem_bytes, stream, __VA_ARGS__); break;        \
        case 2: hipLaunchKernelGGL((KERNEL<4, 2>), g__, b__, smem_bytes, stream, __VA_ARGS__); break;        \
        case 4: hipLaunchKernelGGL((KERNEL<4, 4>), g__, b__, smem_bytes, stream, __VA_ARGS__); break;        \
        case 5: hipLaunchKernelGGL((KERNEL<4, 5>), g__, b__, smem_bytes, stream, __VA_ARGS__); break;        \
        default: hipLaunchKernelGGL((KERNEL<4, 8>), g__, b__, smem_bytes, stream, __VA_ARGS__); break;       \
      }                                                                                                      \
    } else {                                                                                                 \
      switch ((cfg).maxj) {                                                                                  \
        case 1: hipLaunchKernelGGL((KERNEL<1, 1>), g__, b__, smem_bytes, stream, __VA_ARGS__); break;        \
        case 2: hipLaunchKernelGGL((KERNEL<1, 2>), g__, b__, smem_bytes, stream, __VA_ARGS__); break;        \
        case 4: hipLaunchKernelGGL((KERNEL<1, 4>), g__, b__, smem_bytes, stream, __VA_ARGS__); break;        \
        case 8: hipLaunchKernelGGL((KERNEL<1, 8>), g__, b__, smem_bytes, stream, __VA_ARGS__); break;        \
        case 16: hipLaunchKernelGGL((KERNEL<1, 16>), g__, b__, smem_bytes, stream, __VA_ARGS__); break;      \
        default: hipLaunchKernelGGL((KERNEL<1, 32>), g__, b__, smem_bytes, stream, __VA_ARGS__); break;      \
      }                                                                                                      \
    }                                                                                                        \
  } while (0)

#define DISPATCH_COL_Y(KERNEL, cfg, ny, smem_bytes, stream, ...)                                                   \
  do {                                                                                                       \
    dim3 g__((cfg).blocks, (ny)), b__(CGC_BLOCK);                                                                    \
    if ((cfg).vec == 4) {                                                                                    \
      switch ((cfg).maxj) {                                                                                  \
        case 1: hipLaunchKernelGGL((KERNEL<4, 1>), g__, b__, smem_bytes, stream, __VA_ARGS__); break;        \
        case 2: hipLaunchKernelGGL((KERNEL<4, 2>), g__, b__, smem_bytes, stream, __VA_ARGS__); break;        \
        case 4: hipLaunchKernelGGL((KERNEL<4, 4>), g__, b__, smem_bytes, stream, __VA_ARGS__); break;        \
        case 5: hipLaunchKernelGGL((KERNEL<4, 5>), g__, b__, smem_bytes, stream, __VA_ARGS__); break;        \
        default: hipLaunchKernelGGL((KERNEL<4, 8>), g__, b__, smem_bytes, stream, __VA_ARGS__); break;       \
      }                                                                                                      \
    } else {                                                                                                 \
      switch ((cfg).maxj) {                                                                                  \
        case 1: hipLaunchKernelGGL((KERNEL<1, 1>), g__, b__, smem_bytes, stream, __VA_ARGS__); break;        \
        case 2: hipLaunchKernelGGL((KERNEL<1, 2>), g__, b__, smem_bytes, stream, __VA_ARGS__); break;        \
        case 4: hipLaunchKernelGGL((KERNEL<1, 4>), g__, b__, smem_bytes, stream, __VA_ARGS__); break;        \
        case 8: hipLaunchKernelGGL((KERNEL<1, 8>), g__, b__, smem_bytes, stream, __VA_ARGS__); break;        \
        case 16: hipLaunchKernelGGL((KERNEL<1, 16>), g__, b__, smem_bytes, stream, __VA_ARGS__); break;      \
        default: hipLaunchKernelGGL((KERNEL<1, 32>), g__, b__, smem_bytes, stream, __VA_ARGS__); break;      \
      }                                                                                                      \
    }                                                                                                        \
// ... 407 lines not shown
    const int normalize = HOT ? 1 : normalize_rt;
    for (int base = rg.gwave * rg.rpw; base < n; base += rg.nwaves * rg.rpw) {
      const int row = min(base + rg.sub, n - 1);
      const bool valid = base + rg.sub < n;
      Vec<VEC> g[MAXJ], x[MAXJ];
      float dot = 0.f;
  #pragma unroll
      for (int j = 0; j < MAXJ; ++j) {
        const int c = min((rg.sl + lpr * j) * VEC, F - VEC);
        load_wide<VEC, MAXJ>(g[j], dy + (size_t)row * ldy + c);
        load_wide<VEC, MAXJ>(x[j], hn + (size_t)row * F + c);
      }
  #pragma unroll
      for (int j = 0; j < MAXJ; ++j) {
        const int c = (rg.sl + lpr * j) * VEC;
        if (valid && c < F) {
          Vec<VEC> pa, pb, pc, pm, pi;
          if (!REGC && mode != 0) {
            pa.load(lc + c);
            if (mode == 2) { pb.load(lc + F + c); pc.load(lc + 2 * F + c); pm.load(lc + 3 * F + c); pi.load(lc + 4 * F + c); }
          }
  #pragma unroll
          for (int v = 0; v < VEC; ++v) {
            const float xv = x[j].v[v];
            float a_, b_ = 0.f, c_ = 0.f, m_ = 0.f, i_ = 0.f;
            if (REGC) {
              a_ = ca[REGC ? j : 0][REGC ? v : 0]; b_ = cb[REGC ? j : 0][REGC ? v : 0]; c_ = cc[REGC ? j : 0][REGC ? v : 0];
              m_ = mu[REGC ? j : 0][REGC ? v : 0]; i_ = is[REGC ? j : 0][REGC ? v : 0];
            } else if (mode != 0) {
              a_ = pa.v[v];
              if (mode == 2) { b_ = pb.v[v]; c_ = pc.v[v]; m_ = pm.v[v]; i_ = pi.v[v]; }
            } else {
              a_ = 1.f;
            }
            float go = a_ * g[j].v[v];
            if (mode == 2) go = go - b_ - (act_fwd(xv, ACT) - m_) * i_ * c_;
            go *= act_bwd(xv, ACT);
            g[j].v[v] = go;
            dot += xv * go;
          }
        } else {
  #pragma unroll
          for (int v = 0; v < VEC; ++v) g[j].v[v] = x[j].v[v] = 0.f;
        }
      }
      if (normalize) dot = group_sum(dot, lpr);
      if (!valid) continue;
      const float r = normalize ? rinv[row] : 1.f;
      const bool clamped = normalize && !(r < 1.f / L2_EPS);
  #pragma unroll
      for (int j = 0; j < MAXJ; ++j) {
        const int c = (rg.sl + lpr * j) * VEC;
        if (c < F) {
          Vec<VEC> o;
  #pragma unroll
          for (int v = 0; v < VEC; ++v) {
            const float gv = g[j].v[v];
            o.v[v] = !normalize ? gv : (clamped ? gv * (1.f / L2_EPS) : r * (gv - x[j].v[v] * dot));
            csum[0][j][v] += o.v[v];
          }
          o.store(dh + (size_t)row * F + c);
        }
      }
    }
  };
  if (mode == 2 && normalize) {
    switch (act) {
      case CGC_ACT_RELU: rows(std::integral_constant<int, CGC_ACT_RELU>(), std::true_type()); break;
      case CGC_ACT_ELU: rows(std::integral_constant<int, CGC_ACT_ELU>(), std::true_type()); break;
      case CGC_ACT_LEAKYRELU: rows(std::integral_constant<int, CGC_ACT_LEAKYRELU>(), std::true_type()); break;
      default: rows(std::integral_constant<int, CGC_ACT_IDENTITY>(), std::true_type()); break;
    }
  } else {
    switch (act) {
      case CGC_ACT_RELU: rows(std::integral_constant<int, CGC_ACT_RELU>(), std::false_type()); break;
      case CGC_ACT_ELU: rows(std::integral_constant<int, CGC_ACT_ELU>(), std::false_type()); break;
      case CGC_ACT_LEAKYRELU: rows(std::integral_constant<int, CGC_ACT_LEAKYRELU>(), std::false_type()); break;
      default: rows(std::integral_constant<int, CGC_ACT_IDENTITY>(), std::false_type()); break;
    }
  }
  if (ws != nullptr) col_reduce_store<VEC, MAXJ, 1>(csum, F, lpr, smem, ws + (size_t)blockIdx.x * F);
}

extern "C" int cgc_bn_act_l2_bwd(const float* dy, int ldy, const float* hn, const float* rinv, int n, int F, int act,
                                 int normalize, int mode, const float* mean, const float* istd, const float* gamma,
                                 const float* sums, double count, float* dh, float* dh_colsum, float* ws, cgc_stream_t stream) {
  if (F <= 0) return 0;
  if (n <= 0) {
    if (dh_colsum) (void)hipMemsetAsync(dh_colsum, 0, sizeof(float) * F, as_stream(stream));
    return 0;
  }
  if (dh_colsum != nullptr && ws == nullptr) return CGC_EINVAL;
  const bool vec = (F % 4 == 0) && (ldy % 4 == 0) && aligned16(dy) && aligned16(hn) && aligned16(dh);
  ColCfg cfg = col_cfg(n, F, vec);
  if (!cfg.ok) return CGC_EINVAL;
  if (dh_colsum == nullptr) cfg.blocks = row_blocks(n, cfg.lpr);
  const float inv_count = (float)(1.0 / count);
  const size_t smem = sizeof(float) * (3 + 5) * F;
  DISPATCH_COL(k_bn_act_l2_bwd, cfg, smem, as_stream(stream), dy, ldy, hn, rinv, n, F, cfg.lpr, act, normalize, mode, mean, istd,
               gamma, sums, inv_count, dh, dh_colsum ? ws : (float*)nullptr);
  CGC_RETURN_IF_LAUNCH_FAILED();
  if (dh_colsum) {
    hipLaunchKernelGGL(k_reduce_slots<float>, REDUCE_SLOTS_GRID(F), dim3(32 * RS_GROUPS), 0, as_stream(stream), ws, cfg.blocks, F, dh_colsum);
    CGC_RETURN_IF_LAUNCH_FAILED();
  }
  return 0;
}

template <int VEC, int MAXJ>
__global__ __launch_bounds__(256) void k_colsum(const float* __restrict__ x, int ld, int n, int F, int lpr, float* __restrict__ ws) {
  extern __shared__ __attribute__((aligned(16))) float smem[];
  const RowGroup rg(lpr);
  float acc[1][MAXJ][VEC];
#pragma unroll
  for (int j = 0; j < MAXJ; ++j)
#pragma unroll
    for (int v = 0; v < VEC; ++v) acc[0][j][v] = 0.f;
  for (int base = rg.gwave * rg.rpw; base < n; base += rg.nwaves * rg.rpw) {
    const int row = base + rg.sub;
    if (row < n) {
#pragma unroll
      for (int j = 0; j < MAXJ; ++j) {
        const int c = (rg.sl + lpr * j) * VEC;
        if (c < F) {
          Vec<VEC> d;
          d.load(x + (size_t)row * ld + c);
#pragma unroll
          for (int v = 0; v < VEC; ++v) acc[0][j][v] += d.v[v];
        }
      }
    }
  }
  col_reduce_store<VEC, MAXJ, 1>(acc, F, lpr, smem, ws + (size_t)blockIdx.x * F);
}

extern "C" int cgc_colsum(const float* x, int ld, int n, int F, float* out, float* ws, cgc_stream_t stream) {
  if (F <= 0) return 0;
  if (n <= 0) {
    (void)hipMemsetAsync(out, 0, sizeof(float) * F, as_stream(stream));
    return 0;
  }
  const bool vec_ok = (F % 4 == 0) && (ld % 4 == 0) && aligned16(x);
  ColCfg cfg = col_cfg(n, F, vec_ok);
  if (!cfg.ok) return CGC_EINVAL;
  const size_t smem = sizeof(float) * 3 * F;
  DISPATCH_COL(k_colsum, cfg, smem, as_stream(stream), x, ld, n, F, cfg.lpr, ws);
  CGC_RETURN_IF_LAUNCH_FAILED();
  hipLaunchKernelGGL(k_reduce_slots<float>, REDUCE_SLOTS_GRID(F), dim3(32 * RS_GROUPS), 0, as_stream(stream), ws, cfg.blocks, F, out);
  CGC_RETURN_IF_LAUNCH_FAILED();
  return 0;
}

template <int VEC>
__global__ __launch_bounds__(256) void k_softmax_fwd(const float* __restrict__ x, int n, int C, int ld, int lpr, float* __restrict__ out) {
  const RowGroup rg(lpr);
  for (int base = rg.gwave * rg.rpw; base < n; base += rg.nwaves * rg.rpw) {
    const int row = base + rg.sub;
    const bool valid = row < n;
    const float* xr = x + (size_t)row * ld;
    float m = -INFINITY;
    if (valid)
      for (int c = rg.sl * VEC; c < C; c += lpr * VEC) {
        Vec<VEC> t;
        t.load(xr + c);
#pragma unroll
        for (int v = 0; v < VEC; ++v) m = fmaxf(m, t.v[v]);
      }
    m = group_max(m, lpr);
    float s = 0.f;
    if (valid)
      for (int c = rg.sl * VEC; c < C; c += lpr * VEC) {
        Vec<VEC> t;
        t.load(xr + c);
#pragma unroll
        for (int v = 0; v < VEC; ++v) s += expf(t.v[v] - m);
      }
    s = group_sum(s, lpr);
    if (!valid) continue;
    const float inv = 1.f / s;
    for (int c = rg.sl * VEC; c < C; c += lpr * VEC) {
      Vec<VEC> t;
      t.load(xr + c);
#pragma unroll
      for (int v = 0; v < VEC; ++v) t.v[v] = expf(t.v[v] - m) * inv;
      t.store(out + (size_t)row * ld + c);
    }
  }
}

// ... 34 lines not shown
    const float inv = 1.f / s;
#pragma unroll
    for (int j = 0; j < MAXJ; ++j) {
      const int c = (rg.sl + lpr * j) * VEC;
      if (c < C) {
#pragma unroll
        for (int v = 0; v < VEC; ++v) t[j].v[v] *= inv;
        t[j].store(out + (size_t)row * ld + c);
      }
    }
  }
}

template <int VEC, int MAXJ>
__global__ __launch_bounds__(256) void k_softmax_bwd(const float* __restrict__ S, const float* __restrict__ dS, int n, int C,
                                                     int ld, int lpr, float* __restrict__ dx, float* __restrict__ ws) {
  extern __shared__ __attribute__((aligned(16))) float smem[];
  const RowGroup rg(lpr);
  float csum[1][MAXJ][VEC];
#pragma unroll
  for (int j = 0; j < MAXJ; ++j)
#pragma unroll
    for (int v = 0; v < VEC; ++v) csum[0][j][v] = 0.f;
  for (int base = rg.gwave * rg.rpw; base < n; base += rg.nwaves * rg.rpw) {
    const int row = min(base + rg.sub, n - 1);
    const bool valid = base + rg.sub < n;
    Vec<VEC> s[MAXJ], d[MAXJ];
    float dot = 0.f;
#pragma unroll
    for (int j = 0; j < MAXJ; ++j) {
      const int c = min((rg.sl + lpr * j) * VEC, C - VEC);
      load_wide<VEC, MAXJ>(s[j], S + (size_t)row * ld + c);
      load_wide<VEC, MAXJ>(d[j], dS + (size_t)row * ld + c);
    }
#pragma unroll
    for (int j = 0; j < MAXJ; ++j) {
      const bool ok = valid && (rg.sl + lpr * j) * VEC < C;
#pragma unroll
      for (int v = 0; v < VEC; ++v) {
        s[j].v[v] = ok ? s[j].v[v] : 0.f;
        d[j].v[v] = ok ? d[j].v[v] : 0.f;
        dot += s[j].v[v] * d[j].v[v];
      }
    }
    dot = group_sum(dot, lpr);
    if (!valid) continue;
#pragma unroll
    for (int j = 0; j < MAXJ; ++j) {
      const int c = (rg.sl + lpr * j) * VEC;
      if (c < C) {
#pragma unroll
        for (int v = 0; v < VEC; ++v) {
          d[j].v[v] = s[j].v[v] * (d[j].v[v] - dot);
          csum[0][j][v] += d[j].v[v];
        }
        d[j].store(dx + (size_t)row * ld + c);
      }
    }
  }
  if (ws != nullptr) col_reduce_store<VEC, MAXJ, 1>(csum, C, lpr, smem, ws + (size_t)blockIdx.x * C);
}

extern "C" int cgc_softmax_fwd(const float* x, int n, int C, int ld, float* out, cgc_stream_t stream) {
  if (n <= 0 || C <= 0) return 0;
  if (ld < C) return CGC_EINVAL;
  const bool vec = (C % 4 == 0) && (ld % 4 == 0) && aligned16(x) && aligned16(out);
  ColCfg cfg = col_cfg(n, C, vec);
  if (cfg.ok && cfg.maxj <= 8) {
    cfg.blocks = row_blocks(n, cfg.lpr);
    DISPATCH_COL(k_softmax_fwd_reg, cfg, 0, as_stream(stream), x, n, C, ld, cfg.lpr, out);
    CGC_RETURN_IF_LAUNCH_FAILED();
    return 0;
  }
  const int lpr = pick_lpr(vec ? C / 4 : C);
  dim3 grid(row_blocks(n, lpr)), block(CGC_BLOCK);
  if (vec)
    hipLaunchKernelGGL(k_softmax_fwd<4>, grid, block, 0, as_stream(stream), x, n, C, ld, lpr, out);
  else
    hipLaunchKernelGGL(k_softmax_fwd<1>, grid, block, 0, as_stream(stream), x, n, C, ld, lpr, out);
  CGC_RETURN_IF_LAUNCH_FAILED();
  return 0;
}

extern "C" int cgc_softmax_bwd(const float* S, const float* dS, int n, int C, int ld, float* dx, float* dx_colsum, float* ws,
                               cgc_stream_t stream) {
  if (C <= 0) return 0;
  if (ld < C) return CGC_EINVAL;
  if (n <= 0) {
    if (dx_colsum) (void)hipMemsetAsync(dx_colsum, 0, sizeof(float) * C, as_stream(stream));
    return 0;
  }
  if (dx_colsum != nullptr && ws == nullptr) return CGC_EINVAL;
  const bool vec = (C % 4 == 0) && (ld % 4 == 0) && aligned16(S) && aligned16(dS) && aligned16(dx);
  ColCfg cfg = col_cfg(n, C, vec);
  if (!cfg.ok) return CGC_EINVAL;
  if (dx_colsum == nullptr) cfg.blocks = row_blocks(n, cfg.lpr);
  const size_t smem = dx_colsum ? sizeof(float) * 3 * C : 0;
  DISPATCH_COL(k_softmax_bwd, cfg, smem, as_stream(stream), S, dS, n, C, ld, cfg.lpr, dx, dx_colsum ? ws : (float*)nullptr);
  CGC_RETURN_IF_LAUNCH_FAILED();
  if (dx_colsum) {
    hipLaunchKernelGGL(k_reduce_slots<float>, REDUCE_SLOTS_GRID(C), dim3(32 * RS_GROUPS), 0, as_stream(stream), ws, cfg.blocks, C, dx_colsum);
    CGC_RETURN_IF_LAUNCH_FAILED();
  }
  return 0;
}

#define SEGMAX_WAVES 16
__global__ __launch_bounds__(64 * SEGMAX_WAVES) void k_segment_max_fwd(const float* __restrict__ x, const int* __restrict__ gptr,
                                                                       int D, int nmax, float* __restrict__ out,
                                                                       int* __restrict__ arg) {
  __shared__ float bv[SEGMAX_WAVES][64];
  __shared__ int bi[SEGMAX_WAVES][64];
  const int b = blockIdx.x;
  const int lane = threadIdx.x & 63, wave = threadIdx.x >> 6;
  int dp = 64;
  if (D <= 32) dp = D <= 2 ? 2 : D <= 4 ? 4 : D <= 8 ? 8 : D <= 16 ? 16 : 32;
  const int rpw = 64 / dp, sub = lane / dp, dl = lane - sub * dp;
  const int d = blockIdx.y * 64 + dl;
  const int lo = gptr[b], hi = gptr[b + 1];
  float best = -INFINITY;
  int idx = -1;
  if (d < D) {
    const int stride = SEGMAX_WAVES * rpw;
    int r = lo + wave * rpw + sub;
    for (; r + 3 * stride < hi; r += 4 * stride) {
      float v[4];
#pragma unroll
      for (int u = 0; u < 4; ++u) v[u] = x[(size_t)(r + u * stride) * D + d];
#pragma unroll
      for (int u = 0; u < 4; ++u)
        if (v[u] > best) { best = v[u]; idx = r + u * stride; }
    }
    for (; r < hi; r += stride) {
      const float v = x[(size_t)r * D + d];
      if (v > best) { best = v; idx = r; }
    }
  }
  bv[wave][lane] = best;
  bi[wave][lane] = idx;
  __syncthreads();
  if (wave == 0 && sub == 0 && d < D) {
    for (int w = 0; w < SEGMAX_WAVES; ++w)
      for (int s2 = (w == 0 ? 1 : 0); s2 < rpw; ++s2) {
        const float v = bv[w][s2 * dp + dl];
        const int i = bi[w][s2 * dp + dl];
        if (i >= 0 && (v > best || (v == best && i < idx) || idx < 0)) { best = v; idx = i; }
      }
    if (idx < 0) { best = 0.f; }
    else if (hi - lo < nmax && best < 0.f) { best = 0.f; idx = -1; }
    out[(size_t)b * D + d] = best;
    arg[(size_t)b * D + d] = idx;
  }
}

__global__ void k_segment_max_bwd(const float* __restrict__ dout, const int* __restrict__ arg, int total, int D, float* __restrict__ dx) {
  const int i = blockIdx.x * blockDim.x + threadIdx.x;
  if (i >= total) return;
  const int a = arg[i];
  if (a >= 0) dx[(size_t)a * D + (i % D)] = dout[i];
}

extern "C" int cgc_segment_max_fwd(const float* x, const int* gptr, int B, int D, int nmax, float* out, int* arg, cgc_stream_t stream) {
  if (B <= 0 || D <= 0) return 0;
  hipLaunchKernelGGL(k_segment_max_fwd, dim3(B, ceil_div(D, 64)), dim3(64 * SEGMAX_WAVES), 0, as_stream(stream), x, gptr, D, nmax, out, arg);
  CGC_RETURN_IF_LAUNCH_FAILED();
  return 0;
}

__global__ void k_segment_max_bwd_full(const float* __restrict__ dout, const int* __restrict__ arg, const int* __restrict__ gptr, int D,
                                       float* __restrict__ dx) {
  const int b = blockIdx.y;
  const int g0 = gptr[b], cnt = (gptr[b + 1] - g0) * D;
  for (int i = blockIdx.x * blockDim.x + threadIdx.x; i < cnt; i += gridDim.x * blockDim.x) {
    const int r = i / D, d = i - r * D;
    dx[(size_t)g0 * D + i] = (arg[b * D + d] == g0 + r) ? dout[b * D + d] : 0.f;
  }
}

extern "C" int cgc_segment_max_bwd_full(const float* dout, const int* arg, const int* gptr, int B, int D, int nmax, float* dx,
                                        cgc_stream_t stream) {
  if (B <= 0 || D <= 0 || nmax <= 0) return 0;
  if (B > 65535) return CGC_EINVAL;
  int bx = ceil_div(nmax * D, 256 * 4);
  if (bx < 1) bx = 1;
  hipLaunchKernelGGL(k_segment_max_bwd_full, dim3(bx, B), dim3(256), 0, as_stream(stream), dout, arg, gptr, D, dx);
  CGC_RETURN_IF_LAUNCH_FAILED();
  return 0;
// ... 441 lines not shown
```

cgc-net_amd/csrc/sagenarrow.hip:

```cpp
#include "common.hpp"
#include "groups.hpp"

#define L2_EPS 1e-12f
typedef float floatx16 __attribute__((ext_vector_type(16)));

template <int CTRL>
__device__ __forceinline__ float dpp_step(float v) {
  return v + __builtin_bit_cast(float, __builtin_amdgcn_mov_dpp(__builtin_bit_cast(int, v), CTRL, 0xF, 0xF, true));
}
__device__ __forceinline__ float half_sum(float v) {
  v = dpp_step<0xB1>(v);
  v = dpp_step<0x4E>(v);
  v = dpp_step<0x141>(v);
  v = dpp_step<0x140>(v);
  return v + __shfl_xor(v, 16);
}

#define SN_LDT 33

template <int FS, int ACT>
__global__ __launch_bounds__(256) void k_sage_narrow_bwd(const SnBwdPtrs p0, const SnBwdPtrs p1, int ldy, int n, int F, int ,
                                                         int normalize, int mode, float inv_count, int lda, int fin, int ldd, int tiles) {
  const bool second = blockIdx.y != 0;
  const float* __restrict__ dy = second ? p1.dy : p0.dy;
// ... 39 lines not shown
    float dh[16], ag[16];
#pragma unroll
    for (int s = 0; s < 16; ++s) {
      const int row = row0 + 2 * s + half;
      const bool ok = row < n;
      const size_t rc = ok ? row : n - 1;
      const float g_ = dy[rc * ldy + fcl], x_ = hn[rc * F + fcl], a_ = agg[rc * lda + facl];
      const float g = (ok && fok) ? g_ : 0.f;
      const float x = (ok && fok) ? x_ : 0.f;
      ag[s] = (ok && f < fin) ? a_ : 0.f;
      float go = ca * g;
      if (mode == 2) go = go - cb - (act_fwd(x, ACT) - mu) * is * cc;
      go *= act_bwd(x, ACT);
      if (!(ok && fok)) go = 0.f;
      float o = go;
      if (normalize) {
        const float dot = half_sum(x * go);
        const float r_ = rinv[rc];
        const float r = ok ? r_ : 1.f;
        const bool clamped = !(r < 1.f / L2_EPS);
        o = clamped ? go * (1.f / L2_EPS) : r * (go - x * dot);
      }
      dh[s] = o;
      db += o;
    }
#pragma unroll
    for (int s = 0; s < 16; ++s) dw = __builtin_amdgcn_mfma_f32_32x32x2f32(ag[s], dh[s], dw, 0, 0, 0);
    if (dagg != nullptr) {
#pragma unroll
      for (int s = 0; s < 16; ++s) st[(2 * s + half) * SN_LDT + f] = dh[s];
      __builtin_amdgcn_wave_barrier();
      floatx16 da;
#pragma unroll
      for (int r = 0; r < 16; ++r) da[r] = 0.f;
#pragma unroll
      for (int t = 0; t < FS; ++t) da = __builtin_amdgcn_mfma_f32_32x32x2f32(st[f * SN_LDT + 2 * t + half], wb[t], da, 0, 0, 0);
      __builtin_amdgcn_wave_barrier();
      if (f < fin) {
        if (row0 + 32 <= n) {
#pragma unroll
          for (int r = 0; r < 16; ++r) dagg[(size_t)(row0 + (r & 3) + 8 * (r >> 2) + 4 * half) * ldd + f] = da[r];
        } else {
#pragma unroll
          for (int r = 0; r < 16; ++r) {
            const int row = row0 + (r & 3) + 8 * (r >> 2) + 4 * half;
            if (row < n) dagg[(size_t)row * ldd + f] = da[r];
          }
        }
      }
    }
  }
  __syncthreads();
  float* __restrict__ xch = &strip[0][0];
  static_assert(32 * SN_LDT <= 17 * 64, "transposition strip exceeds the per-wave LDS");
#pragma unroll
  for (int r = 0; r < 16; ++r) xch[(wave * 17 + r) * 64 + lane] = dw[r];
  xch[(wave * 17 + 16) * 64 + lane] = db;
  __syncthreads();
  if (wave == 0) {
    float* __restrict__ slot = ws + (size_t)blockIdx.x * (fin * F + F);
#pragma unroll
    for (int r = 0; r < 16; ++r) {
      const float v = (xch[(0 * 17 + r) * 64 + lane] + xch[(1 * 17 + r) * 64 + lane]) + (xch[(2 * 17 + r) * 64 + lane] + xch[(3 * 17 + r) * 64 + lane]);
      const int k = (r & 3) + 8 * (r >> 2) + 4 * half;
      if (fok && k < fin) slot[k * F + f] = v;
    }
    float d = (xch[(0 * 17 + 16) * 64 + lane] + xch[(1 * 17 + 16) * 64 + lane]) + (xch[(2 * 17 + 16) * 64 + lane] + xch[(3 * 17 + 16) * 64 + lane]);
    d += __shfl_xor(d, 32);
    if (fok && half == 0) slot[fin * F + f] = d;
  }
}

int launch_reduce_slots_f32(const float* ws, int slots, int width, float* out, hipStream_t stream);

static int sn_grid(int n) {
  const int tiles = ceil_div(n, 32);
  int g = ceil_div(tiles, 4);
  return g < 1024 ? g : 1024;
}

extern "C" int64_t cgc_sage_narrow_ws_floats(int n, int fin, int F) { return (int64_t)sn_grid(n > 0 ? n : 1) * (fin * F + F); }

int sage_narrow_bwd_groups(const SnBwdPtrs* g, float* const* dwdb, int ng, int ldy, int n, int F, int act, int normalize, int mode, double count,
                           int lda, int fin, int ldd, hipStream_t st) {
  if (F <= 0 || fin <= 0) return 0;
  if (F > 32 || fin > 32 || ng < 1 || ng > 2) return CGC_EINVAL;
  for (int i = 0; i < ng; ++i)
    if (g[i].ws == nullptr || dwdb[i] == nullptr || (g[i].dagg != nullptr && ldd < fin)) return CGC_EINVAL;
  const int width = fin * F + F;
  if (n <= 0) {
    for (int i = 0; i < ng; ++i) (void)hipMemsetAsync(dwdb[i], 0, sizeof(float) * width, st);
    return 0;
  }
  const int tiles = ceil_div(n, 32), grid = sn_grid(n);
  const float inv_count = (float)(1.0 / count);
  const int fs = (F + 1) / 2;
  const SnBwdPtrs& g1 = g[ng - 1];
#define SN_LAUNCH(FS_, ACT_)                                                                                                       \
  hipLaunchKernelGGL((k_sage_narrow_bwd<FS_, ACT_>), dim3(grid, ng), dim3(256), 0, st, g[0], g1, ldy, n, F, act, normalize, mode, inv_count, \
                     lda, fin, ldd, tiles)
#define SN_ACT(FS_)                                                                                        \
  switch (act) {                                                                                           \
    case CGC_ACT_RELU: SN_LAUNCH(FS_, CGC_ACT_RELU); break;                                                \
    case CGC_ACT_ELU: SN_LAUNCH(FS_, CGC_ACT_ELU); break;                                                  \
    case CGC_ACT_LEAKYRELU: SN_LAUNCH(FS_, CGC_ACT_LEAKYRELU); break;                                      \
    default: SN_LAUNCH(FS_, CGC_ACT_IDENTITY); break;                                                      \
  }
  if (fs <= 8) { SN_ACT(8); } else if (fs <= 10) { SN_ACT(10); } else { SN_ACT(16); }
#undef SN_ACT
#undef SN_LAUNCH
  CGC_RETURN_IF_LAUNCH_FAILED();
  return launch_reduce_slots_f32_pair(g[0].ws, dwdb[0], g1.ws, dwdb[ng - 1], ng, grid, width, st);
}

extern "C" int cgc_sage_narrow_bwd(const float* dy, int ldy, const float* hn, const float* rinv, int n, int F, int act, int normalize,
                                   int mode, const float* mean, const float* istd, const float* gamma, const float* sums, double count,
                                   const float* agg, int lda, int fin, const float* W, float* dagg, int ldd, float* dwdb, float* ws,
                                   cgc_stream_t stream_) {
  const SnBwdPtrs g{dy, hn, rinv, mean, istd, gamma, sums, agg, W, dagg, ws};
  float* const out[1] = {dwdb};
  return sage_narrow_bwd_groups(&g, out, 1, ldy, n, F, act, normalize, mode, count, lda, fin, ldd, as_stream(stream_));
}

template <int KS, int ACT>
__global__ __launch_bounds__(256) void k_sage_narrow_fwd(const SnFwdPtrs p0, const SnFwdPtrs p1, int lda, int n, int K, int F, int normalize,
                                                         int , int tiles) {
  const bool second = blockIdx.y != 0;
  const float* __restrict__ agg = second ? p1.agg : p0.agg;
  const float* __restrict__ W = second ? p1.W : p0.W;
  const float* __restrict__ bias = second ? p1.bias : p0.bias;
  float* __restrict__ hn = second ? p1.hn : p0.hn;
  float* __restrict__ rinv_out = second ? p1.rinv : p0.rinv;
  float* __restrict__ ws = second ? p1.ws : p0.ws;
  __shared__ double xch[4][2][32];
  const int lane = threadIdx.x & 63, wave = threadIdx.x >> 6;
  const int f = lane & 31, half = lane >> 5;
  const bool fok = f < F;
  float bw[KS];
#pragma unroll
  for (int s = 0; s < KS; ++s) {
    const int k = 2 * s + half;
    bw[s] = (fok && k < K) ? W[(size_t)k * F + f] : 0.f;
  }
  const float bia = (fok && bias != nullptr) ? bias[f] : 0.f;
  double s1 = 0.0, s2 = 0.0;
  for (int tile = blockIdx.x * 4 + wave; tile < tiles; tile += gridDim.x * 4) {
    const int row0 = tile * 32;
    const float* __restrict__ a = agg + (size_t)min(row0 + f, n - 1) * lda;
    float av[KS];
#pragma unroll
    for (int s = 0; s < KS; ++s) {
      const int k = 2 * s + half;
      const float ld = a[k < K ? k : 0];
      av[s] = k < K ? ld : 0.f;
    }
    floatx16 acc;
#pragma unroll
    for (int r = 0; r < 16; ++r) acc[r] = bia;
#pragma unroll
    for (int s = 0; s < KS; ++s) acc = __builtin_amdgcn_mfma_f32_32x32x2f32(av[s], bw[s], acc, 0, 0, 0);
    float vv[16], rr[16];
#pragma unroll
    for (int r = 0; r < 16; ++r) {
      float v = fok ? acc[r] : 0.f;
      float rin = 1.f;
      if (normalize) {
        const float q = half_sum(v * v);
        rin = 1.f / fmaxf(sqrtf(q), L2_EPS);
        v *= rin;
      }
      vv[r] = v;
      rr[r] = rin;
    }
    if (row0 + 32 <= n) {
      if (fok) {
#pragma unroll
        for (int r = 0; r < 16; ++r) {
          const int row = row0 + (r & 3) + 8 * (r >> 2) + 4 * half;
          const double o = (double)act_fwd(vv[r], ACT);
          s1 += o;
          s2 = fma(o, o, s2);
          hn[(size_t)row * F + f] = vv[r];
        }
      }
      if (f == 0) {
#pragma unroll
        for (int r = 0; r < 16; ++r) rinv_out[row0 + (r & 3) + 8 * (r >> 2) + 4 * half] = rr[r];
      }
    } else {
#pragma unroll
      for (int r = 0; r < 16; ++r) {
        const int row = row0 + (r & 3) + 8 * (r >> 2) + 4 * half;
        if (row < n) {
          if (fok) {
            const double o = (double)act_fwd(vv[r], ACT);
            s1 += o;
            s2 = fma(o, o, s2);
            hn[(size_t)row * F + f] = vv[r];
          }
          if (f == 0) rinv_out[row] = rr[r];
        }
      }
    }
  }
// ... 63 lines not shown
```

Before: 2796 graphs/s.

## Defer gradient slot reductions into one batched finish kernel per level backward

Instead of launching a separate reduction kernel after each backward op (sage narrow bwd, bn/act bwd, softmax bwd, split-K GEMM, JK LSTM partial fold), the partial-sum workspaces are kept live in a new deferred arena. Descriptors are queued and drained by a single multi-descriptor k_grad_finish launch at the end of each level's backward. This is meant to cut many small kernel launches and their serialization. In exchange it uses more scratch memory, since workspaces can no longer be released right away, and adds a dry-run pass to size the deferred arena. The batch-sum reduction loop is also unrolled by eight.

After: 2810 graphs/s (median of 6 runs). No clear change (+0.5%).

```diff
diff --git a/cgc-net_amd/csrc/exec.hip b/cgc-net_amd/csrc/exec.hip
--- a/cgc-net_amd/csrc/exec.hip
+++ b/cgc-net_amd/csrc/exec.hip
@@ -4,6 +4,8 @@
 
 #include "common.hpp"
 #include "groups.hpp"
+#include "finish.hpp"
+#include "jk.hpp"
 
 struct CatArgs {
   const float* src[4];
@@ -70,7 +72,40 @@
   return 0;
 }
 
-int reduce_batch_sum_rows(const float* ws, float* out, int parts, int rows, int width, int ldo, float beta, hipStream_t stream);
+__global__ __launch_bounds__(1024) void k_grad_finish(const FinishArgs a, int n) {
+  __shared__ double part[RS_GROUPS][32];
+  int i = 0, first = 0;
+#pragma unroll
+  for (int k = 1; k < FIN_MAX; ++k)
+    if (k < n && (int)blockIdx.x >= a.start[k]) {
+      i = k;
+      first = a.start[k];
+    }
+  const FinishDesc& d = a.d[i];
+  const int bx = blockIdx.x - first;
+  if (bx >= d.blocks) return;
+  switch (d.kind) {
+    case FIN_SLOTS:
+      reduce_slots_body<float, float>(d.src, d.count, d.numel, d.dst, bx, part);
+      break;
+    case FIN_MANY_PARTS: {
+      const int sub = threadIdx.x >> 8;
+      reduce_many_parts_body(d.src, d.dst, d.count, d.numel, d.beta, d.width, d.ld, bx * 4 + sub, threadIdx.x & 255,
+                             reinterpret_cast<float(*)[32]>(&part[0][0]) + sub * 8);
+      break;
+    }
+    case FIN_BATCH_SUM:
+      reduce_batch_sum_body(d.src, d.dst, d.count, d.numel, d.beta, d.width, d.ld, bx * 1024ll + threadIdx.x, d.blocks * 1024ll);
+      break;
+    default: {
+      const int nbx = (d.numel + 1023) / 1024, p2 = bx / nbx;
+      jk_pg_fold_body(d.src, d.count, d.width, d.numel, d.dst, (bx - p2 * nbx) * 1024 + (int)threadIdx.x, p2, 0);
+      break;
+    }
+  }
+}
+
+int reduce_batch_sum_desc(const float* ws, float* out, int parts, int rows, int width, int ldo, float beta, FinishDesc* d);
 
 namespace {
 
@@ -97,6 +132,14 @@
   float* gws;
   int64_t gws_floats;
   int gemm_mode = CGC_GEMM_EXACT;
+  Arena* defer = nullptr;
+  struct Finish* fin = nullptr;
+};
+
+struct Finish {
+  FinishArgs a;
+  int n = 0;
+  JkPending jk{};
 };
 
 static int fail_at(int rc, const char* what, int line) {
@@ -116,6 +159,42 @@
     const int rc__ = (expr);                                    \
     if (rc__ != 0) return fail_at(rc__, #expr, __LINE__);       \
   } while (0)
+
+int finish_flush(const Ctx& c) {
+  Finish& f = *c.fin;
+  if (f.n > 0) {
+    FinishDesc bulk[FIN_MAX];
+    int nb = 0, nk = 0;
+    for (int i = 0; i < f.n; ++i) {
+      if (f.a.d[i].kind == FIN_BATCH_SUM) bulk[nb++] = f.a.d[i];
+      else f.a.d[nk++] = f.a.d[i];
+    }
+    for (int i = 0; i < nb; ++i) f.a.d[nk + i] = bulk[i];
+    int blocks = 0;
+    for (int i = 0; i < f.n; ++i) {
+      f.a.start[i] = blocks;
+      blocks += f.a.d[i].blocks;
+    }
+    hipLaunchKernelGGL(k_grad_finish, dim3((unsigned)blocks), dim3(1024), 0, as_stream(c.s), f.a, f.n);
+    CGC_RETURN_IF_LAUNCH_FAILED();
+    f.n = 0;
+  }
+  if (f.jk.P > 0) {
+    TRY(jk_finish_flat(f.jk, as_stream(c.s)));
+    f.jk.P = 0;
+  }
+  return 0;
+}
+int defer_push(const Ctx& c, const FinishDesc& d) {
+  if (c.dry || d.blocks <= 0) return 0;
+  if (c.fin->n == FIN_MAX) TRY(finish_flush(c));
+  c.fin->a.d[c.fin->n++] = d;
+  return 0;
+}
+int defer_slots(const Ctx& c, const float* ws, int slots, int width, float* out) {
+  if (slots <= 0) return 0;
+  return defer_push(c, FinishDesc{ws, out, FIN_SLOTS, slots, width, width, width, (width + 31) / 32, 0.f, 0});
+}
 
 inline int up(int v, int m) { return (v + m - 1) / m * m; }
 inline int wide_ld(int F) { return (F >= 256 && F % 32 != 0) ? up(F, 32) : (F > 32 && F % 4 != 0) ? up(F, 4) : F; }
@@ -164,12 +243,11 @@
   if (parts == 1) return gemm(c, 1, 0, Fa, Fb, n, A, lda, B, ldb, 0.f, out, ldo);
   const int chunk = up(ceil_div(n, parts), 32);
   parts = ceil_div(n, chunk);
-  const size_t m = c.scratch->mark();
-  float* ws = c.scratch->f((size_t)parts * Fa * Fb);
+  float* ws = c.defer->f((size_t)parts * Fa * Fb);
   TRY(gemm(c, 1, 0, Fa, Fb, n, A, lda, B, ldb, 0.f, ws, Fb, nullptr, parts, 0, 0, (int64_t)Fa * Fb, nullptr, 3, chunk));
-  CALL(reduce_batch_sum_rows(ws, out, parts, Fa, Fb, ldo, 0.f, as_stream(c.s)));
-  c.scratch->release(m);
-  return 0;
+  FinishDesc fd{};
+  CALL(reduce_batch_sum_desc(ws, out, parts, Fa, Fb, ldo, 0.f, &fd));
+  return defer_push(c, fd);
 }
 
 struct T3 {
@@ -284,14 +362,18 @@
   }
   float* db = d.has_bias ? dwdb + (size_t)fin * F : nullptr;
   if (F <= 32 && fin <= 32) {
-    float* ws = c.scratch->f((size_t)cgc_sage_narrow_ws_floats(n, fin, F));
-    CALL(cgc_sage_narrow_bwd(dy, ldy, s.hn, s.rinv, n, F, d.act, 1, mode, s.mean, s.istd, p.gamma, d.has_bn ? sums : nullptr, d.count, agg,
-                             lda, fin, p.W, dagg, ldd, dwdb, ws, c.s));
+    const SnBwdPtrs g{dy, s.hn, s.rinv, s.mean, s.istd, p.gamma, d.has_bn ? sums : nullptr, agg, p.W, dagg,
+                      c.defer->f((size_t)cgc_sage_narrow_ws_floats(n, fin, F))};
+    int slots = 0;
+    CALL(sage_narrow_bwd_groups(&g, &dwdb, 1, ldy, n, F, d.act, 1, mode, d.count, lda, fin, ldd, as_stream(c.s), &slots));
+    TRY(defer_slots(c, g.ws, slots, fin * F + F, dwdb));
   } else {
     float* dh = c.scratch->f((size_t)n * F);
-    float* ws = db ? c.scratch->f(slot_floats) : nullptr;
-    CALL(cgc_bn_act_l2_bwd(dy, ldy, s.hn, s.rinv, n, F, d.act, 1, mode, s.mean, s.istd, p.gamma, d.has_bn ? sums : nullptr, d.count, dh, db, ws,
-                           c.s));
+    float* ws = db ? c.defer->f(slot_floats) : nullptr;
+    int slots = 0;
+    CALL(bn_act_l2_bwd_slots(dy, ldy, s.hn, s.rinv, n, F, d.act, 1, mode, s.mean, s.istd, p.gamma, d.has_bn ? sums : nullptr, d.count, dh, db, ws,
+                             c.s, &slots));
+    TRY(defer_slots(c, ws, slots, F, db));
     if (dagg) TRY(gemm(c, 0, 1, n, fin, F, dh, F, p.W, F, 0.f, dagg, ldd));
     TRY(gemm_tn_rows(c, agg, lda, fin, dh, F, F, n, dwdb));
   }
@@ -335,8 +417,10 @@
   SnBwdPtrs g[2];
   for (int i = 0; i < 2; ++i)
     g[i] = SnBwdPtrs{dy[i], s[i].hn, s[i].rinv, s[i].mean, s[i].istd, p[i].gamma, d.has_bn ? sums[i] : nullptr, agg[i], p[i].W, dagg[i],
-                     c.scratch->f((size_t)cgc_sage_narrow_ws_floats(n, fin, F))};
-  CALL(sage_narrow_bwd_groups(g, dwdb, 2, ldy, n, F, d.act, 1, mode, d.count, lda, fin, ldd, as_stream(c.s)));
+                     c.defer->f((size_t)cgc_sage_narrow_ws_floats(n, fin, F))};
+  int slots = 0;
+  CALL(sage_narrow_bwd_groups(g, dwdb, 2, ldy, n, F, d.act, 1, mode, d.count, lda, fin, ldd, as_stream(c.s), &slots));
+  for (int i = 0; i < 2; ++i) TRY(defer_slots(c, g[i].ws, slots, fin * F + F, dwdb[i]));
   c.scratch->release(m);
   return 0;
 }
@@ -587,10 +671,14 @@
   float* d_cat = d_embed;
   if (d.jk) {
     d_cat = sc.f((size_t)n * D3);
-    const size_t m = sc.mark();
-    float* ws = sc.f((size_t)cgc_jk_bwd_ws_floats(H));
-    CALL(cgc_jk_lstm_bwd_flat(L.cat_e, d_embed, n, L.npad_jk, H, jk->lstm, jk->w_att, jk->b_att, L.HS, L.CS, d_cat, grads + L.gl.jk, ws, c.s));
-    sc.release(m);
+    float* ws = c.defer->f((size_t)cgc_jk_bwd_ws_floats(H));
+    if (!c.dry) {
+      JkPending& pj = c.fin->jk;
+      TRY(jk_lstm_bwd_flat_deferred(L.cat_e, d_embed, n, L.npad_jk, H, jk->lstm, jk->w_att, jk->b_att, L.HS, L.CS, d_cat, grads + L.gl.jk, ws, c.s,
+                                    &pj));
+      if (pj.P > 0)
+        TRY(defer_push(c, FinishDesc{pj.ws, pj.tmp, FIN_JK_FOLD, pj.P, pj.per, pj.P2, 0, ceil_div(pj.per, 1024) * pj.P2, 0.f, 0}));
+    }
   }
   float* dagg[2];
   const int ldg = L.ldp;
@@ -643,9 +731,9 @@
   return 0;
 }
 
-int level_bwd(const Ctx& c, Level& L, const cgc_block_params* emb, const cgc_block_params* pl, const cgc_jk_params* jk, const cgc_graph* g,
-              const int* gptr, const float* x_in, const float* A_in, const float* d_readout, const float* d_xo, const float* d_ao, float* grads,
-              float* d_x_in, float* d_A_in, const float* d_reg = nullptr) {
+int level_bwd_body(const Ctx& c, Level& L, const cgc_block_params* emb, const cgc_block_params* pl, const cgc_jk_params* jk, const cgc_graph* g,
+                   const int* gptr, const float* x_in, const float* A_in, const float* d_readout, const float* d_xo, const float* d_ao,
+                   float* grads, float* d_x_in, float* d_A_in, const float* d_reg) {
   const cgc_level_desc& d = L.d;
   Arena& sc = *c.scratch;
   const int n = L.n, H = L.H, AH = L.AH, wp = L.wp, C = L.C, D = L.D, B = L.B, R = L.R;
@@ -693,10 +781,10 @@
     if (L.reg) CALL(cgc_diffpool_reg_entropy_bwd(L.S, n, C, L.ldC, coef, ds, L.ldC, c.s));
     float* dz = sc.f((size_t)n * L.ldC);
     {
-      const size_t m = sc.mark();
-      float* ws = sc.f((size_t)(cgc_stats_blocks(n, C) > 1 ? cgc_stats_blocks(n, C) : 1) * 2 * C);
-      CALL(cgc_softmax_bwd(L.S, ds, n, C, L.ldC, dz, grads + L.gl.lin_b, ws, c.s));
-      sc.release(m);
+      float* ws = c.defer->f((size_t)(cgc_stats_blocks(n, C) > 1 ? cgc_stats_blocks(n, C) : 1) * 2 * C);
+      int slots = 0;
+      CALL(softmax_bwd_slots(L.S, ds, n, C, L.ldC, dz, grads + L.gl.lin_b, ws, c.s, &slots));
+      TRY(defer_slots(c, ws, slots, C, grads + L.gl.lin_b));
     }
     dx12 = sc.f((size_t)n * 2 * AH);
     float* dy3 = sc.f((size_t)n * L.ldC);
@@ -714,6 +802,27 @@
     return level_bwd_blocks(c, L, emb, pl, jk, g, gptr, x_in, A_in, d_embed, dx12, dagg1, gAt, grads, d_x_in, d_A_in);
   }
   return level_bwd_blocks(c, L, emb, pl, jk, g, gptr, x_in, A_in, d_embed, nullptr, nullptr, nullptr, grads, d_x_in, d_A_in);
+}
+
+int level_bwd(const Ctx& c, Level& L, const cgc_block_params* emb, const cgc_block_params* pl, const cgc_jk_params* jk, const cgc_graph* g,
+              const int* gptr, const float* x_in, const float* A_in, const float* d_readout, const float* d_xo, const float* d_ao, float* grads,
+              float* d_x_in, float* d_A_in, const float* d_reg = nullptr) {
+  TRY(level_bwd_body(c, L, emb, pl, jk, g, gptr, x_in, A_in, d_readout, d_xo, d_ao, grads, d_x_in, d_A_in, d_reg));
+  return c.dry ? 0 : finish_flush(c);
+}
+
+int64_t deferred_floats(Level& L) {
+  Arena sc(nullptr), df(nullptr);
+  Ctx c{nullptr, true, &sc, nullptr, 0};
+  c.defer = &df;
+  cgc_block_params bp;
+  memset(&bp, 0, sizeof(bp));
+  cgc_jk_params jp;
+  memset(&jp, 0, sizeof(jp));
+  cgc_graph gr;
+  memset(&gr, 0, sizeof(gr));
+  if (level_bwd(c, L, &bp, &bp, &jp, &gr, nullptr, nullptr, nullptr, nullptr, nullptr, nullptr, nullptr, nullptr, nullptr) != 0) return -1;
+  return (int64_t)df.high;
 }
 
 template <class Body>
@@ -767,9 +876,15 @@
   L.layout_grads();
   size_t high = 0;
   for (int pass = 0; pass < (d->eval ? 1 : 2); ++pass) {
-    Arena sc(nullptr);
+    Arena sc(nullptr), df(nullptr);
     Ctx c{nullptr, true, &sc, nullptr, 0};
+    c.defer = &df;
     sc.f((size_t)cgc_gemm_ws_floats());
+    if (pass == 1) {
+      const int64_t deferred = deferred_floats(L);
+      if (deferred < 0) return -1;
+      sc.f((size_t)deferred);
+    }
     cgc_block_params bp;
     memset(&bp, 0, sizeof(bp));
     cgc_jk_params jp;
@@ -806,7 +921,13 @@
   if (!cgc_level_supported(d) || saved == nullptr || scratch == nullptr || grads == nullptr || d->eval) return CGC_EINVAL;
   if (!aligned16(saved) || !aligned16(scratch) || !aligned16(grads)) return CGC_EINVAL;
   if ((d->flags & 8) && d_reg == nullptr) return CGC_EINVAL;
-  return run_level(d, const_cast<float*>(saved), scratch, stream, [&](const Ctx& c, Level& L) {
+  return run_level(d, const_cast<float*>(saved), scratch, stream, [&](Ctx& c, Level& L) {
+    const int64_t deferred = deferred_floats(L);
+    if (deferred < 0) return CGC_EINVAL;
+    Arena df(c.scratch->f((size_t)deferred));
+    Finish fin;
+    c.defer = &df;
+    c.fin = &fin;
     return level_bwd(c, L, emb, pool, jk, g, gptr, x_in, A_in, d_readout, d_x_out, d_A_out, grads, d_x_in, d_A_in, d_reg);
   });
 }
diff --git a/cgc-net_amd/csrc/finish.hpp b/cgc-net_amd/csrc/finish.hpp
--- /dev/null
+++ b/cgc-net_amd/csrc/finish.hpp
@@ -0,0 +1,107 @@
+#pragma once
+#include "common.hpp"
+
+#define RS_GROUPS 32
+template <typename OUT, typename IN>
+__device__ __forceinline__ void reduce_slots_body(const IN* __restrict__ ws, int slots, int width, OUT* __restrict__ out, int bx,
+                                                  double (*part)[32]) {
+  const int cl = threadIdx.x & 31, grp = threadIdx.x >> 5;
+  const int c = bx * 32 + cl;
+  double s = 0.0;
+  if (c < width) {
+    double a[4] = {0.0, 0.0, 0.0, 0.0};
+    int k = grp;
+    for (; k + 3 * RS_GROUPS < slots; k += 4 * RS_GROUPS) {
+#pragma unroll
+      for (int u = 0; u < 4; ++u) a[u] += (double)ws[(size_t)(k + RS_GROUPS * u) * width + c];
+    }
+    for (; k < slots; k += RS_GROUPS) a[0] += (double)ws[(size_t)k * width + c];
+    s = (a[0] + a[1]) + (a[2] + a[3]);
+  }
+  part[grp][cl] = s;
+  __syncthreads();
+  if (grp == 0 && c < width) {
+    double t[4] = {0.0, 0.0, 0.0, 0.0};
+#pragma unroll
+    for (int g = 0; g < RS_GROUPS; g += 4) { t[0] += part[g][cl]; t[1] += part[g + 1][cl]; t[2] += part[g + 2][cl]; t[3] += part[g + 3][cl]; }
+    out[c] = (OUT)((t[0] + t[1]) + (t[2] + t[3]));
+  }
+}
+
+__device__ __forceinline__ void reduce_many_parts_body(const float* __restrict__ ws, float* __restrict__ out, int parts, int numel, float beta,
+                                                       int width, int ldo, int bx, int tid, float (*part)[32]) {
+  const int cl = tid & 31, grp = tid >> 5;
+  const int c = bx * 32 + cl;
+  float s = 0.f;
+  if (c < numel) {
+    float a[8];
+#pragma unroll
+    for (int u = 0; u < 8; ++u) a[u] = 0.f;
+    int k = grp;
+    for (; k + 56 < parts; k += 64) {
+#pragma unroll
+      for (int u = 0; u < 8; ++u) a[u] += ws[(size_t)(k + 8 * u) * numel + c];
+    }
+    for (; k < parts; k += 8) a[0] += ws[(size_t)k * numel + c];
+    s = ((a[0] + a[1]) + (a[2] + a[3])) + ((a[4] + a[5]) + (a[6] + a[7]));
+  }
+  part[grp][cl] = s;
+  __syncthreads();
+  if (grp == 0 && c < numel) {
+    float t = part[0][cl];
+#pragma unroll
+    for (int g = 1; g < 8; ++g) t += part[g][cl];
+    const int o = (c / width) * ldo + c % width;
+    out[o] = beta != 0.f ? t + beta * out[o] : t;
+  }
+}
+
+__device__ __forceinline__ void reduce_batch_sum_body(const float* __restrict__ ws, float* __restrict__ out, int parts, long long numel,
+                                                      float beta, int width, int ldo, long long first, long long stride) {
+  for (long long i = first; i < numel; i += stride) {
+    float s = 0.f;
+    for (int p = 0; p < parts; p += 8) {
+      float v[8];
+#pragma unroll
+      for (int u = 0; u < 8; ++u) v[u] = p + u < parts ? ws[(size_t)(p + u) * numel + i] : 0.f;
+#pragma unroll
+      for (int u = 0; u < 8; ++u)
+        if (p + u < parts) s += v[u];
+    }
+    const long long o = (i / width) * ldo + i % width;
+    out[o] = beta != 0.f ? s + beta * out[o] : s;
+  }
+}
+
+__device__ __forceinline__ void jk_pg_fold_body(const float* __restrict__ part, int P, int P2, int per, float* __restrict__ tmp, int e, int p2,
+                                                int d) {
+  if (e >= per) return;
+  const float* src = part + ((size_t)d * P + (size_t)p2 * 16) * per + e;
+  const int cnt = min(16, P - p2 * 16);
+  float v[16];
+#pragma unroll
+  for (int k = 0; k < 16; ++k) v[k] = k < cnt ? src[(size_t)k * per] : 0.f;
+  float a = 0.f;
+#pragma unroll
+  for (int k = 0; k < 16; ++k)
+    if (k < cnt) a += v[k];
+  tmp[((size_t)d * P2 + p2) * per + e] = a;
+}
+
+enum { FIN_SLOTS = 0, FIN_MANY_PARTS = 1, FIN_BATCH_SUM = 2, FIN_JK_FOLD = 3 };
+struct FinishDesc {
+  const float* src;
+  float* dst;
+  int kind;
+  int count;
+  int numel;
+  int width, ld;
+  int blocks;
+  float beta;
+  int pad_;
+};
+#define FIN_MAX 16
+struct FinishArgs {
+  int start[FIN_MAX];
+  FinishDesc d[FIN_MAX];
+};
diff --git a/cgc-net_amd/csrc/gemm.hip b/cgc-net_amd/csrc/gemm.hip
--- a/cgc-net_amd/csrc/gemm.hip
+++ b/cgc-net_amd/csrc/gemm.hip
@@ -1,4 +1,5 @@
 #include "gemm_common.hpp"
+#include "finish.hpp"
 
 template <int ROWS>
 struct KContigLoader {
@@ -649,43 +650,15 @@
 
 __global__ void k_reduce_batch_sum(const float* __restrict__ ws, float* __restrict__ out, int parts, long long numel, float beta, int width,
                                    int ldo) {
-  for (long long i = blockIdx.x * (long long)blockDim.x + threadIdx.x; i < numel; i += (long long)gridDim.x * blockDim.x) {
-    float s = 0.f;
-    for (int p = 0; p < parts; ++p) s += ws[(size_t)p * numel + i];
-    const long long o = (i / width) * ldo + i % width;
-    out[o] = beta != 0.f ? s + beta * out[o] : s;
-  }
+  reduce_batch_sum_body(ws, out, parts, numel, beta, width, ldo, blockIdx.x * (long long)blockDim.x + threadIdx.x,
+                        (long long)gridDim.x * blockDim.x);
 }
 
 __global__ __launch_bounds__(256) void k_reduce_many_parts(const float* __restrict__ ws, float* __restrict__ out, int parts, int numel,
                                                            float beta, int width, int ldo) {
   __shared__ float part[8][32];
-  const int cl = threadIdx.x & 31, grp = threadIdx.x >> 5;
-  const int c = blockIdx.x * 32 + cl;
-  ws += (size_t)blockIdx.y * parts * numel;
-  out += (size_t)blockIdx.y * numel;
-  float s = 0.f;
-  if (c < numel) {
-    float a[8];
-#pragma unroll
-    for (int u = 0; u < 8; ++u) a[u] = 0.f;
-    int k = grp;
-    for (; k + 56 < parts; k += 64) {
-#pragma unroll
-      for (int u = 0; u < 8; ++u) a[u] += ws[(size_t)(k + 8 * u) * numel + c];
-    }
-    for (; k < parts; k += 8) a[0] += ws[(size_t)k * numel + c];
-    s = ((a[0] + a[1]) + (a[2] + a[3])) + ((a[4] + a[5]) + (a[6] + a[7]));
-  }
-  part[grp][cl] = s;
-  __syncthreads();
-  if (grp == 0 && c < numel) {
-    float t = part[0][cl];
-#pragma unroll
-    for (int g = 1; g < 8; ++g) t += part[g][cl];
-    const int o = (c / width) * ldo + c % width;
-    out[o] = beta != 0.f ? t + beta * out[o] : t;
-  }
+  reduce_many_parts_body(ws + (size_t)blockIdx.y * parts * numel, out + (size_t)blockIdx.y * numel, parts, numel, beta, width, ldo,
+                         blockIdx.x, threadIdx.x, part);
 }
 
 extern "C" int cgc_reduce_batched(const float* ws, float* out, int outer, int parts, int numel, float beta, cgc_stream_t stream) {
@@ -697,19 +670,17 @@
   return 0;
 }
 
-int reduce_batch_sum_rows(const float* ws, float* out, int parts, int rows, int width, int ldo, float beta, hipStream_t stream) {
+int reduce_batch_sum_desc(const float* ws, float* out, int parts, int rows, int width, int ldo, float beta, FinishDesc* d) {
+  *d = FinishDesc{};
   const int64_t numel = (int64_t)rows * width;
   if (numel <= 0) return 0;
   if (width <= 0 || ldo < width || numel > 0x7fffffff) return CGC_EINVAL;
   if (parts >= 16 && numel <= (1 << 20)) {
-    hipLaunchKernelGGL(k_reduce_many_parts, dim3((unsigned)ceil_div((int)numel, 32), 1u), dim3(256), 0, stream, ws, out, parts, (int)numel, beta,
-                       width, ldo);
+    *d = FinishDesc{ws, out, FIN_MANY_PARTS, parts, (int)numel, width, ldo, ceil_div(ceil_div((int)numel, 32), 4), beta, 0};
   } else {
-    const int64_t blocks = ceil_div64(numel, 256);
-    hipLaunchKernelGGL(k_reduce_batch_sum, dim3((unsigned)(blocks < 4096 ? blocks : 4096)), dim3(256), 0, stream, ws, out, parts,
-                       (long long)numel, beta, width, ldo);
-  }
-  CGC_RETURN_IF_LAUNCH_FAILED();
+    const int64_t blocks = ceil_div64(numel, 1024);
+    *d = FinishDesc{ws, out, FIN_BATCH_SUM, parts, (int)numel, width, ldo, (int)(blocks < 1024 ? blocks : 1024), beta, 0};
+  }
   return 0;
 }
 
diff --git a/cgc-net_amd/csrc/groups.hpp b/cgc-net_amd/csrc/groups.hpp
--- a/cgc-net_amd/csrc/groups.hpp
+++ b/cgc-net_amd/csrc/groups.hpp
@@ -34,8 +34,14 @@
 int sage_narrow_fwd_groups(const SnFwdPtrs* g, const SnFwdBn* bn, int ng, int lda, int n, int K, int F, int normalize, int act, int stats,
                            double count, hipStream_t st);
 int sage_narrow_bwd_groups(const SnBwdPtrs* g, float* const* dwdb, int ng, int ldy, int n, int F, int act, int normalize, int mode, double count,
-                           int lda, int fin, int ldd, hipStream_t st);
+                           int lda, int fin, int ldd, hipStream_t st, int* slots_out = nullptr);
 int bn_act_apply_groups(const BnApplyPtrs* g, int ng, int n, int F, int act, int ldy, hipStream_t stream);
 int bn_bwd_reduce_groups(const BnRedPtrs* g, float* const* sums, int ng, int ldy, int n, int F, int act, hipStream_t stream);
 int launch_stats_finalize_groups(const StatsFinPtrs* g, int ng, int slots, int F, double count, hipStream_t stream);
 int launch_reduce_slots_f32_pair(const float* ws0, float* out0, const float* ws1, float* out1, int ng, int slots, int width, hipStream_t stream);
+
+int bn_act_l2_bwd_slots(const float* dy, int ldy, const float* hn, const float* rinv, int n, int F, int act, int normalize, int mode,
+                        const float* mean, const float* istd, const float* gamma, const float* sums, double count, float* dh,
+                        float* dh_colsum, float* ws, cgc_stream_t stream, int* slots_out);
+int softmax_bwd_slots(const float* S, const float* dS, int n, int C, int ld, float* dx, float* dx_colsum, float* ws, cgc_stream_t stream,
+                      int* slots_out);
diff --git a/cgc-net_amd/csrc/jk.hip b/cgc-net_amd/csrc/jk.hip
--- a/cgc-net_amd/csrc/jk.hip
+++ b/cgc-net_amd/csrc/jk.hip
@@ -361,6 +361,17 @@
   return jk_mfma_bwd_flat(xs, dout, n, npad, C, w, HS, CS, dxs, flat, ws, as_stream(stream));
 }
 
+int jk_lstm_bwd_flat_deferred(const float* xs, const float* dout, int n, int npad, int C, const float* const* lstm, const float* w_att,
+                              const float* b_att, const float* HS, const float* CS, float* dxs, float* flat, float* ws, cgc_stream_t stream,
+                              JkPending* pending) {
+  *pending = JkPending{};
+  if (n <= 0) return 0;
+  if (!jk_npad_ok(n, npad)) return CGC_EINVAL;
+  JkWeights w;
+  fill_weights(w, lstm, w_att, b_att);
+  return jk_mfma_bwd_flat(xs, dout, n, npad, C, w, HS, CS, dxs, flat, ws, as_stream(stream), pending);
+}
+
 __global__ void k_jk_unpack(const float* __restrict__ G, int C, int H, float* __restrict__ flat) {
   const int NI = C + 2 * H + 1, NG = 4 * H + 1;
   const int per_dir = 4 * H * C + 4 * H * H + 8 * H, total = 2 * per_dir + 2 * H + 1;
diff --git a/cgc-net_amd/csrc/jk.hpp b/cgc-net_amd/csrc/jk.hpp
--- a/cgc-net_amd/csrc/jk.hpp
+++ b/cgc-net_amd/csrc/jk.hpp
@@ -26,5 +26,14 @@
 int64_t jk_mfma_bwd_ws_floats(int C);
 int jk_mfma_bwd_params(const float* xs, const float* dout, int n, int npad, int C, const JkWeights& w, const float* HS,
                        const float* CS, float* dxs, float* G, float* ws, hipStream_t st);
+struct JkPending {
+  const float* ws;
+  float *tmp, *flat;
+  int P, P2, per, C;
+};
 int jk_mfma_bwd_flat(const float* xs, const float* dout, int n, int npad, int C, const JkWeights& w, const float* HS, const float* CS,
-                     float* dxs, float* flat, float* ws, hipStream_t st);
+                     float* dxs, float* flat, float* ws, hipStream_t st, JkPending* pending = nullptr);
+int jk_lstm_bwd_flat_deferred(const float* xs, const float* dout, int n, int npad, int C, const float* const* lstm, const float* w_att,
+                              const float* b_att, const float* HS, const float* CS, float* dxs, float* flat, float* ws, cgc_stream_t stream,
+                              JkPending* pending);
+int jk_finish_flat(const JkPending& p, hipStream_t st);
diff --git a/cgc-net_amd/csrc/jk_mfma.hip b/cgc-net_amd/csrc/jk_mfma.hip
--- a/cgc-net_amd/csrc/jk_mfma.hip
+++ b/cgc-net_amd/csrc/jk_mfma.hip
@@ -1,4 +1,5 @@
 #include "jk.hpp"
+#include "finish.hpp"
 
 typedef float floatx16 __attribute__((ext_vector_type(16)));
 
@@ -309,13 +310,7 @@
 }
 
 __global__ void k_jk_pg_fold(const float* __restrict__ part, int P, int P2, int per, float* __restrict__ tmp) {
-  const int e = blockIdx.x * blockDim.x + threadIdx.x, p2 = blockIdx.y, d = blockIdx.z;
-  if (e >= per) return;
-  const float* src = part + ((size_t)d * P + (size_t)p2 * 16) * per + e;
-  const int cnt = min(16, P - p2 * 16);
-  float a = 0.f;
-  for (int k = 0; k < cnt; ++k) a += src[(size_t)k * per];
-  tmp[((size_t)d * P2 + p2) * per + e] = a;
+  jk_pg_fold_body(part, P, P2, per, tmp, blockIdx.x * blockDim.x + threadIdx.x, blockIdx.y, blockIdx.z);
 }
 
 template <int C>
@@ -862,8 +857,16 @@
 }
 
 template <int C>
+static int launch_finish_flat(const JkPending& p, hipStream_t st) {
+  constexpr int H = JkU<C>::H, total = 2 * (4 * H * C + 4 * H * H + 8 * H) + 2 * H + 1;
+  hipLaunchKernelGGL(k_jku_finish_flat<C>, dim3(ceil_div(total, 128)), dim3(128), 0, st, p.tmp, p.P2, p.flat);
+  CGC_RETURN_IF_LAUNCH_FAILED();
+  return 0;
+}
+
+template <int C>
 static int launch_bwd_params(const float* xs, const float* dout, int n, int npad, const JkWeights& w, const float* HS, const float* CS,
-                             float* dxs, float* G, float* ws, hipStream_t st, float* flat) {
+                             float* dxs, float* G, float* ws, hipStream_t st, float* flat, JkPending* pending = nullptr) {
   constexpr size_t lds = sizeof(float) * JkU<C>::BWD_TOTAL;
   static bool attr_set[CGC_MAX_DEVICES] = {};
   cgc_allow_lds(reinterpret_cast<const void*>(&k_jku_bwd<C>), (int)lds, attr_set);
@@ -874,10 +877,13 @@
   constexpr int per = JkU<C>::PG_FLOATS, H = JkU<C>::H;
   const int P = grid, P2 = ceil_div(P, 16);
   float* tmp = ws + (size_t)P * per;
+  if (pending != nullptr) {
+    *pending = JkPending{ws, tmp, flat, P, P2, per, C};
+    return 0;
+  }
   hipLaunchKernelGGL(k_jk_pg_fold, dim3(ceil_div(per, 256), P2, 1), dim3(256), 0, st, ws, P, P2, per, tmp);
   if (flat != nullptr) {
-    constexpr int total = 2 * (4 * H * C + 4 * H * H + 8 * H) + 2 * H + 1;
-    hipLaunchKernelGGL(k_jku_finish_flat<C>, dim3(ceil_div(total, 128)), dim3(128), 0, st, tmp, P2, flat);
+    return launch_finish_flat<C>(JkPending{ws, tmp, flat, P, P2, per, C}, st);
   } else {
     constexpr int total = 2 * (4 * H + 1) * (C + 2 * H + 1);
     hipLaunchKernelGGL(k_jku_finish_G<C>, dim3(ceil_div(total, 128)), dim3(128), 0, st, tmp, P2, G);
@@ -908,15 +914,26 @@
 }
 
 int jk_mfma_bwd_flat(const float* xs, const float* dout, int n, int npad, int C, const JkWeights& w, const float* HS, const float* CS,
-                     float* dxs, float* flat, float* ws, hipStream_t st) {
+                     float* dxs, float* flat, float* ws, hipStream_t st, JkPending* pending) {
   if ((reinterpret_cast<uintptr_t>(xs) & 15u) || (reinterpret_cast<uintptr_t>(dout) & 15u) || (reinterpret_cast<uintptr_t>(dxs) & 15u))
     return CGC_EINVAL;
   switch (C) {
-    case 4: return launch_bwd_params<4>(xs, dout, n, npad, w, HS, CS, dxs, nullptr, ws, st, flat);
-    case 8: return launch_bwd_params<8>(xs, dout, n, npad, w, HS, CS, dxs, nullptr, ws, st, flat);
-    case 12: return launch_bwd_params<12>(xs, dout, n, npad, w, HS, CS, dxs, nullptr, ws, st, flat);
-    case 16: return launch_bwd_params<16>(xs, dout, n, npad, w, HS, CS, dxs, nullptr, ws, st, flat);
-    case 20: return launch_bwd_params<20>(xs, dout, n, npad, w, HS, CS, dxs, nullptr, ws, st, flat);
+    case 4: return launch_bwd_params<4>(xs, dout, n, npad, w, HS, CS, dxs, nullptr, ws, st, flat, pending);
+    case 8: return launch_bwd_params<8>(xs, dout, n, npad, w, HS, CS, dxs, nullptr, ws, st, flat, pending);
+    case 12: return launch_bwd_params<12>(xs, dout, n, npad, w, HS, CS, dxs, nullptr, ws, st, flat, pending);
+    case 16: return launch_bwd_params<16>(xs, dout, n, npad, w, HS, CS, dxs, nullptr, ws, st, flat, pending);
+    case 20: return launch_bwd_params<20>(xs, dout, n, npad, w, HS, CS, dxs, nullptr, ws, st, flat, pending);
+    default: return CGC_EINVAL;
+  }
+}
+
+int jk_finish_flat(const JkPending& p, hipStream_t st) {
+  switch (p.C) {
+    case 4: return launch_finish_flat<4>(p, st);
+    case 8: return launch_finish_flat<8>(p, st);
+    case 12: return launch_finish_flat<12>(p, st);
+    case 16: return launch_finish_flat<16>(p, st);
+    case 20: return launch_finish_flat<20>(p, st);
     default: return CGC_EINVAL;
   }
 }
diff --git a/cgc-net_amd/csrc/rowops.hip b/cgc-net_amd/csrc/rowops.hip
--- a/cgc-net_amd/csrc/rowops.hip
+++ b/cgc-net_amd/csrc/rowops.hip
@@ -2,6 +2,7 @@
 
 #include "common.hpp"
 #include "groups.hpp"
+#include "finish.hpp"
 
 #define L2_EPS 1e-12f
 #define RENORM_EPS 1e-15f
@@ -83,60 +84,17 @@
   }
 }
 
-#define RS_GROUPS 32
 template <typename OUT, typename IN = float>
 __global__ __launch_bounds__(32 * RS_GROUPS) void k_reduce_slots(const IN* __restrict__ ws, int slots, int width, OUT* __restrict__ out) {
   __shared__ double part[RS_GROUPS][32];
-  const int cl = threadIdx.x & 31, grp = threadIdx.x >> 5;
-  const int c = blockIdx.x * 32 + cl;
-  double s = 0.0;
-  if (c < width) {
-    double a[4] = {0.0, 0.0, 0.0, 0.0};
-    int k = grp;
-    for (; k + 3 * RS_GROUPS < slots; k += 4 * RS_GROUPS) {
-#pragma unroll
-      for (int u = 0; u < 4; ++u) a[u] += (double)ws[(size_t)(k + RS_GROUPS * u) * width + c];
-    }
-    for (; k < slots; k += RS_GROUPS) a[0] += (double)ws[(size_t)k * width + c];
-    s = (a[0] + a[1]) + (a[2] + a[3]);
-  }
-  part[grp][cl] = s;
-  __syncthreads();
-  if (grp == 0 && c < width) {
-    double t[4] = {0.0, 0.0, 0.0, 0.0};
-#pragma unroll
-    for (int g = 0; g < RS_GROUPS; g += 4) { t[0] += part[g][cl]; t[1] += part[g + 1][cl]; t[2] += part[g + 2][cl]; t[3] += part[g + 3][cl]; }
-    out[c] = (OUT)((t[0] + t[1]) + (t[2] + t[3]));
-  }
+  reduce_slots_body<OUT, IN>(ws, slots, width, out, blockIdx.x, part);
 }
 #define REDUCE_SLOTS_GRID(width) dim3(ceil_div((width), 32))
 
 __global__ __launch_bounds__(32 * RS_GROUPS) void k_reduce_slots_pair(const float* __restrict__ ws0, float* __restrict__ out0,
                                                                      const float* __restrict__ ws1, float* __restrict__ out1, int slots, int width) {
-  const float* __restrict__ ws = blockIdx.y ? ws1 : ws0;
-  float* __restrict__ out = blockIdx.y ? out1 : out0;
   __shared__ double part[RS_GROUPS][32];
-  const int cl = threadIdx.x & 31, grp = threadIdx.x >> 5;
-  const int c = blockIdx.x * 32 + cl;
-  double s = 0.0;
-  if (c < width) {
-    double a[4] = {0.0, 0.0, 0.0, 0.0};
-    int k = grp;
-    for (; k + 3 * RS_GROUPS < slots; k += 4 * RS_GROUPS) {
-#pragma unroll
-      for (int u = 0; u < 4; ++u) a[u] += (double)ws[(size_t)(k + RS_GROUPS * u) * width + c];
-    }
-    for (; k < slots; k += RS_GROUPS) a[0] += (double)ws[(size_t)k * width + c];
-    s = (a[0] + a[1]) + (a[2] + a[3]);
-  }
-  part[grp][cl] = s;
-  __syncthreads();
-  if (grp == 0 && c < width) {
-    double t[4] = {0.0, 0.0, 0.0, 0.0};
-#pragma unroll
-    for (int g = 0; g < RS_GROUPS; g += 4) { t[0] += part[g][cl]; t[1] += part[g + 1][cl]; t[2] += part[g + 2][cl]; t[3] += part[g + 3][cl]; }
-    out[c] = (float)((t[0] + t[1]) + (t[2] + t[3]));
-  }
+  reduce_slots_body<float, float>(blockIdx.y ? ws1 : ws0, slots, width, blockIdx.y ? out1 : out0, blockIdx.x, part);
 }
 int launch_reduce_slots_f32_pair(const float* ws0, float* out0, const float* ws1, float* out1, int ng, int slots, int width, hipStream_t stream) {
   hipLaunchKernelGGL(k_reduce_slots_pair, dim3(ceil_div(width, 32), ng), dim3(32 * RS_GROUPS), 0, stream, ws0, out0, ws1, out1, slots, width);
@@ -710,9 +668,10 @@
   if (ws != nullptr) col_reduce_store<VEC, MAXJ, 1>(csum, F, lpr, smem, ws + (size_t)blockIdx.x * F);
 }
 
-extern "C" int cgc_bn_act_l2_bwd(const float* dy, int ldy, const float* hn, const float* rinv, int n, int F, int act,
-                                 int normalize, int mode, const float* mean, const float* istd, const float* gamma,
-                                 const float* sums, double count, float* dh, float* dh_colsum, float* ws, cgc_stream_t stream) {
+int bn_act_l2_bwd_slots(const float* dy, int ldy, const float* hn, const float* rinv, int n, int F, int act, int normalize, int mode,
+                        const float* mean, const float* istd, const float* gamma, const float* sums, double count, float* dh,
+                        float* dh_colsum, float* ws, cgc_stream_t stream, int* slots_out) {
+  if (slots_out) *slots_out = 0;
   if (F <= 0) return 0;
   if (n <= 0) {
     if (dh_colsum) (void)hipMemsetAsync(dh_colsum, 0, sizeof(float) * F, as_stream(stream));
@@ -728,11 +687,19 @@
   DISPATCH_COL(k_bn_act_l2_bwd, cfg, smem, as_stream(stream), dy, ldy, hn, rinv, n, F, cfg.lpr, act, normalize, mode, mean, istd,
                gamma, sums, inv_count, dh, dh_colsum ? ws : (float*)nullptr);
   CGC_RETURN_IF_LAUNCH_FAILED();
-  if (dh_colsum) {
+  if (dh_colsum && slots_out) {
+    *slots_out = cfg.blocks;
+  } else if (dh_colsum) {
     hipLaunchKernelGGL(k_reduce_slots<float>, REDUCE_SLOTS_GRID(F), dim3(32 * RS_GROUPS), 0, as_stream(stream), ws, cfg.blocks, F, dh_colsum);
     CGC_RETURN_IF_LAUNCH_FAILED();
   }
   return 0;
+}
+
+extern "C" int cgc_bn_act_l2_bwd(const float* dy, int ldy, const float* hn, const float* rinv, int n, int F, int act,
+                                 int normalize, int mode, const float* mean, const float* istd, const float* gamma,
+                                 const float* sums, double count, float* dh, float* dh_colsum, float* ws, cgc_stream_t stream) {
+  return bn_act_l2_bwd_slots(dy, ldy, hn, rinv, n, F, act, normalize, mode, mean, istd, gamma, sums, count, dh, dh_colsum, ws, stream, nullptr);
 }
 
 template <int VEC, int MAXJ>
@@ -933,8 +900,9 @@
   return 0;
 }
 
-extern "C" int cgc_softmax_bwd(const float* S, const float* dS, int n, int C, int ld, float* dx, float* dx_colsum, float* ws,
-                               cgc_stream_t stream) {
+int softmax_bwd_slots(const float* S, const float* dS, int n, int C, int ld, float* dx, float* dx_colsum, float* ws, cgc_stream_t stream,
+                      int* slots_out) {
+  if (slots_out) *slots_out = 0;
   if (C <= 0) return 0;
   if (ld < C) return CGC_EINVAL;
   if (n <= 0) {
@@ -949,11 +917,18 @@
   const size_t smem = dx_colsum ? sizeof(float) * 3 * C : 0;
   DISPATCH_COL(k_softmax_bwd, cfg, smem, as_stream(stream), S, dS, n, C, ld, cfg.lpr, dx, dx_colsum ? ws : (float*)nullptr);
   CGC_RETURN_IF_LAUNCH_FAILED();
-  if (dx_colsum) {
+  if (dx_colsum && slots_out) {
+    *slots_out = cfg.blocks;
+  } else if (dx_colsum) {
     hipLaunchKernelGGL(k_reduce_slots<float>, REDUCE_SLOTS_GRID(C), dim3(32 * RS_GROUPS), 0, as_stream(stream), ws, cfg.blocks, C, dx_colsum);
     CGC_RETURN_IF_LAUNCH_FAILED();
   }
   return 0;
+}
+
+extern "C" int cgc_softmax_bwd(const float* S, const float* dS, int n, int C, int ld, float* dx, float* dx_colsum, float* ws,
+                               cgc_stream_t stream) {
+  return softmax_bwd_slots(S, dS, n, C, ld, dx, dx_colsum, ws, stream, nullptr);
 }
 
 #define SEGMAX_WAVES 16
diff --git a/cgc-net_amd/csrc/sagenarrow.hip b/cgc-net_amd/csrc/sagenarrow.hip
--- a/cgc-net_amd/csrc/sagenarrow.hip
+++ b/cgc-net_amd/csrc/sagenarrow.hip
@@ -145,7 +145,8 @@
 extern "C" int64_t cgc_sage_narrow_ws_floats(int n, int fin, int F) { return (int64_t)sn_grid(n > 0 ? n : 1) * (fin * F + F); }
 
 int sage_narrow_bwd_groups(const SnBwdPtrs* g, float* const* dwdb, int ng, int ldy, int n, int F, int act, int normalize, int mode, double count,
-                           int lda, int fin, int ldd, hipStream_t st) {
+                           int lda, int fin, int ldd, hipStream_t st, int* slots_out) {
+  if (slots_out) *slots_out = 0;
   if (F <= 0 || fin <= 0) return 0;
   if (F > 32 || fin > 32 || ng < 1 || ng > 2) return CGC_EINVAL;
   for (int i = 0; i < ng; ++i)
@@ -173,6 +174,10 @@
 #undef SN_ACT
 #undef SN_LAUNCH
   CGC_RETURN_IF_LAUNCH_FAILED();
+  if (slots_out) {
+    *slots_out = grid;
+    return 0;
+  }
   return launch_reduce_slots_f32_pair(g[0].ws, dwdb[0], g1.ws, dwdb[ng - 1], ng, grid, width, st);
 }
 
@@ -182,7 +187,7 @@
                                    cgc_stream_t stream_) {
   const SnBwdPtrs g{dy, hn, rinv, mean, istd, gamma, sums, agg, W, dagg, ws};
   float* const out[1] = {dwdb};
-  return sage_narrow_bwd_groups(&g, out, 1, ldy, n, F, act, normalize, mode, count, lda, fin, ldd, as_stream(stream_));
+  return sage_narrow_bwd_groups(&g, out, 1, ldy, n, F, act, normalize, mode, count, lda, fin, ldd, as_stream(stream_), nullptr);
 }
 
 template <int KS, int ACT>
```
